# DIAGNijmegen/bodyct-dram-emph-subtype

Measured on NVIDIA B200. Metric: CT volumes/sec med3ddram inference, higher is better.
Workload: dtype f16 operands / f32 accumulate

## Files before the change

### bodyct-dram-emph-subtype_b200/_capi.py

```python
import ctypes as C
import os

HERE = os.path.dirname(os.path.abspath(__file__))
LIB_PATH = os.environ.get("DRAM_B200_LIB") or os.path.join(HERE, "libdram_b200.so")

DRAM_OK = 0
DRAM_DTYPE_BF16 = 0
DRAM_DTYPE_F16 = 1
CONV_ALGO = {"auto": 0, "tiles": 1, "planes": 2}
CONV_EPILOGUE = {"auto": 0, "direct": 1, "staged": 2}
LOSS_COEF_HEAD = 16
PEER_HANDLE_BYTES = 64


class ConvDesc(C.Structure):

    _fields_ = [
        ("n", C.c_int32), ("di", C.c_int32), ("hi", C.c_int32), ("wi", C.c_int32),
        ("c1", C.c_int32), ("c2", C.c_int32),
        ("cout", C.c_int32),
        ("kd", C.c_int32), ("kh", C.c_int32), ("kw", C.c_int32),
        ("sd", C.c_int32), ("sh", C.c_int32), ("sw", C.c_int32),
        ("dd", C.c_int32), ("dh", C.c_int32), ("dw", C.c_int32),
        ("pd", C.c_int32), ("ph", C.c_int32), ("pw", C.c_int32),
        ("relu", C.c_int32),
        ("res_c", C.c_int32), ("res_stride", C.c_int32),
        ("res_d", C.c_int32), ("res_h", C.c_int32), ("res_w", C.c_int32),
        ("n_heads", C.c_int32), ("head_ch", C.c_int32 * 2), ("head_sigmoid", C.c_int32),
        ("store_out", C.c_int32),
        ("tw", C.c_int32), ("th", C.c_int32), ("td", C.c_int32),
        ("dtype", C.c_int32),
        ("algo", C.c_int32),
        ("src1_up2x", C.c_int32),
        ("epilogue", C.c_int32),
    ]


_vp, _i32, _i64, _sz = C.c_void_p, C.c_int32, C.c_int64, C.c_size_t
_pi32 = C.POINTER(C.c_int32)

SIGNATURES = {
    "dram_version": (C.c_int, []),
    "dram_last_error": (C.c_int, [C.c_char_p, _sz]),
    "dram_sm_count": (C.c_int, []),
    "dram_set_saturation_counter": (C.c_int, [_vp]),
    "dram_conv3d_out_dims": (C.c_int, [C.POINTER(ConvDesc), _pi32, _pi32, _pi32]),
    "dram_conv3d_plan_create": (C.c_int, [C.POINTER(ConvDesc), _vp, _vp, _vp, _vp, _vp, _vp, _vp, _vp, _vp,
                                          _vp, _vp, C.POINTER(_vp)]),
    "dram_conv3d_plan_destroy": (C.c_int, [_vp]),
    "dram_conv3d_run": (C.c_int, [_vp, _i32, _vp]),
    "dram_conv3d_plan_info": (C.c_int, [_vp, C.POINTER(_i64), _pi32, _pi32, _pi32, _pi32]),
    "dram_conv3d_plan_executed_flops": (C.c_int, [_vp, C.POINTER(_i64)]),
    "dram_conv3d_worklist_size": (C.c_int, [_vp, _pi32]),
    "dram_conv3d_worklist": (C.c_int, [_vp, _vp, _i32, _vp, _vp, _vp, _vp]),
    "dram_conv3d_run_listed": (C.c_int, [_vp, _vp, _vp, _i32, _vp]),
    "dram_stem_expand": (C.c_int, [_vp, _vp, _i32, _i32, _i32, _i32, _i32, _vp]),
    "dram_stem_weight_bytes": (_sz, []),
    "dram_stem_conv7": (C.c_int, [_vp, _vp, _vp, _vp, _vp, _i32, _i32, _i32, _i32, _i32, _i32, _i32, _vp]),
    "dram_stem_conv7_hu": (C.c_int, [_vp, _vp, _i32, _i32, _vp, _vp, _vp, _vp, _i32, _i32, _i32, _i32, _i32, _i32,
                                     _i32, _vp]),
    "dram_maxpool3d": (C.c_int, [_vp, _vp, _i32, _i32, _i32, _i32, _i32, _i32, _vp]),
    "dram_upsample2x": (C.c_int, [_vp, _vp, _i32, _i32, _i32, _i32, _i32, _i32, _vp]),
    "dram_upsample2x_plan_create": (C.c_int, [_vp, _vp, _i32, _i32, _i32, _i32, _i32, _i32, C.POINTER(_vp)]),
    "dram_upsample2x_plan_destroy": (C.c_int, [_vp]),
    "dram_upsample2x_plan_run": (C.c_int, [_vp, _i32, _vp]),
    "dram_upsample2x_worklist_size": (C.c_int, [_vp, _pi32]),
    "dram_upsample2x_worklist": (C.c_int, [_vp, _vp, _i32, _vp, _vp, _vp, _vp]),
    "dram_upsample2x_plan_run_listed": (C.c_int, [_vp, _vp, _vp, _i32, _vp]),
    "dram_decoder_support": (C.c_int, [_vp, _i32, _i32, _i32, _i32, _i32, _i32, _i32, _vp, _vp, _vp]),
    "dram_upconv_axis": (C.c_int, [_vp, _vp, _i64, _i32, _i32, _i64, _i32, _i32, _i32, _vp]),
    "dram_pool_workspace_bytes": (_sz, [_i32, _i32]),
    "dram_masked_pool": (C.c_int, [_vp, _vp, _i32, _vp, _vp, _i32, _i32, _i32, _i32, _i32, _i32, _i32, _i32, _vp]),
    "dram_dram_workspace_bytes": (_sz, [_i32]),
    "dram_dram_upsample_mask": (C.c_int, [_vp, _vp, _vp, _vp, _vp, _vp, _vp, _vp, _i32, _i32, _i32, _i32,
                                          _i32, _i32, _i32, _i32, _vp]),
    "dram_lobe_workspace_bytes": (_sz, [_i32, _i64]),
    "dram_lobe_sums": (C.c_int, [_vp, _vp, _vp, _vp, _vp, _vp, _vp, _i32, _i64, _vp]),
    "dram_preprocess_workspace_bytes": (_sz, []),
    "dram_window_standardize": (C.c_int, [_vp, _vp, _vp, _vp, _i64, C.c_float, C.c_float, _vp]),
    "dram_preprocess_workspace_bytes_n": (_sz, [_i32]),
    "dram_window_standardize_batch": (C.c_int, [_vp, _vp, _vp, _vp, _i32, _i64, C.c_float, C.c_float, _vp]),
    "dram_window_stats": (C.c_int, [_vp, _vp, _vp, _i32, _i64, C.c_float, C.c_float, _vp]),
    "dram_window_lut": (C.c_int, [_vp, _vp, _vp, _vp, _i32, _i64, C.c_float, C.c_float, _vp]),
    "dram_resize_image": (C.c_int, [_vp, _vp, _vp, _i32, _i32, _i32, _i32, _i32, _i32, _vp]),
    "dram_resize_mask": (C.c_int, [_vp, _vp, _vp, _i32, _i32, _i32, _i32, _i32, _i32, _vp]),
    "dram_resize_labels": (C.c_int, [_vp, _vp, _vp, _i32, _i32, _i32, _i32, _i32, _i32, _vp]),
    "dram_mask_bbox": (C.c_int, [_vp, _i32, _i32, _i32, _vp, _vp]),
    "dram_lung_crop_workspace_bytes": (_sz, [_i32, _i32, _i32]),
    "dram_lung_crop": (C.c_int, [_vp, _vp, _i32, _i32, _i32, _i32, _i32, _i32, _i32, _i32, _i32, _vp, _vp, _vp, _vp, _vp]),
    "dram_label_counts": (C.c_int, [_vp, _i64, _vp, _vp]),
    "dram_label_hu_hist": (C.c_int, [_vp, _vp, _i64, _vp, _i32, _vp, _vp, _vp]),
    "dram_heatmap_u8": (C.c_int, [_vp, _i32, _i32, _i32, _vp, _i32, _i32, _i32, _i32, _i32, _i32, _i32, _i32, _i32, _vp]),
    "dram_conv3d_wgrad_workspace_bytes": (_i64, [C.POINTER(ConvDesc)]),
    "dram_conv3d_wgrad_plan_create": (C.c_int, [C.POINTER(ConvDesc), _vp, _vp, _vp, _i32, _i32, _vp, _i64, C.POINTER(_vp)]),
    "dram_conv3d_wgrad_plan_destroy": (C.c_int, [_vp]),
    "dram_conv3d_wgrad_plan_info": (C.c_int, [_vp, C.POINTER(_i64), _pi32, _pi32, _pi32]),
    "dram_conv3d_wgrad_run": (C.c_int, [_vp, _i32, _i32, _vp]),
    "dram_bn_workspace_bytes": (_i64, [_i32]),
    "dram_bn_stats": (C.c_int, [_vp, _i64, _i32, _i32, _vp, _vp, _vp]),
    "dram_bn_finalize": (C.c_int, [_vp, C.c_double, _vp, _vp, C.c_float, C.c_float, _vp, _vp, _vp, _vp, _vp, _vp, _i32, _vp]),
    "dram_bn_apply": (C.c_int, [_vp, _vp, _vp, _vp, _i32, _vp, _i64, _i32, _i32, _vp]),
    "dram_bn_backward_reduce": (C.c_int, [_vp, _vp, _vp, _vp, _vp, _i64, _i32, _i32, _vp, _vp, _vp]),
    "dram_bn_backward_apply": (C.c_int, [_vp, _vp, _vp, _vp, _vp, _vp, _vp, C.c_double, _vp, _vp, _i64, _i32, _i32, _vp]),
    "dram_upsample2x_backward": (C.c_int, [_vp, _vp, _i32, _i32, _i32, _i32, _i32, _i32, _vp]),
    "dram_maxpool3d_backward_workspace_bytes": (_i64, [_i32, _i32, _i32, _i32, _i32]),
    "dram_maxpool3d_backward": (C.c_int, [_vp, _vp, _vp, _vp, _i32, _i32, _i32, _i32, _i32, _i32, _vp]),
    "dram_heads_workspace_bytes": (_i64, []),
    "dram_heads_sigmoid_forward": (C.c_int, [_vp, _vp, _vp, _vp, _vp, _i64, _i32, _vp]),
    "dram_heads_sigmoid_backward": (C.c_int, [_vp, _vp, _vp, _vp, _vp, _vp, _vp, _vp, _vp, _vp, _i64, _i32, _vp]),
    "dram_peer_exchange_bytes": (_i64, []),
    "dram_peer_alloc": (C.c_int, [_i64, C.POINTER(_vp), _vp]),
    "dram_peer_open": (C.c_int, [_vp, C.POINTER(_vp)]),
    "dram_peer_close": (C.c_int, [_vp]),
    "dram_peer_free": (C.c_int, [_vp]),
    "dram_peer_allreduce_f64": (C.c_int, [_vp, _vp, _i32, _vp, _i32, _i32, C.c_uint64, _vp, _vp]),
    "dram_train_loss_workspace_bytes": (_i64, [_i32]),
    "dram_train_loss_forward": (C.c_int, [_vp, _vp, _vp, _vp, _vp, _vp, _vp, _vp, _vp, _vp, _i32, _i32, _i32, _i32, _i32,
                                          _i32, _i32, C.c_float, C.c_float, _vp, _vp, _vp]),
    "dram_train_loss_backward": (C.c_int, [_vp, _vp, _vp, _vp, _vp, _vp, _vp, _vp, _i32, _i32, _i32, _i32, _i32, _i32,
                                           _i32, _vp, _vp, _vp]),
    "dram_adam_step": (C.c_int, [_vp, _vp, _vp, _vp, _i64, C.c_double, C.c_double, C.c_double, C.c_double, _i32,
                                 C.c_float, _vp]),
    "dram_pack_conv_weight": (C.c_int, [_vp, _vp, _i32, _i32, _i32, _i32, _i32, _i32, _i32, _i32, _vp]),
    "dram_ncdhw_f32_to_ndhwc_16": (C.c_int, [_vp, _vp, _i32, _i32, _i32, _i32, _i32, _i32, _vp]),
    "dram_ndhwc_16_to_ncdhw_f32": (C.c_int, [_vp, _vp, _i32, _i32, _i32, _i32, _i32, _i32, _vp]),
}

_lib = None


class DramError(RuntimeError):
    """A libdram_b200 call returned a negative status."""


def load():
    global _lib
    if _lib is not None:
        return _lib
    if not os.path.exists(LIB_PATH):
        raise ImportError(
            f"{LIB_PATH} is missing: build it with `python {os.path.join(HERE, 'build.py')}` "
            "(there is no CPU or library fallback for this path)")
    lib = C.CDLL(LIB_PATH)
    for name, (res, args) in SIGNATURES.items():
        fn = getattr(lib, name)
        fn.restype = res
        fn.argtypes = args
    _lib = lib
    return lib


def last_error():
    buf = C.create_string_buffer(512)
    load().dram_last_error(buf, len(buf))
    return buf.value.decode("utf-8", "replace")


def check(status, what):
    if status != DRAM_OK:
        raise DramError(f"{what} failed ({status}): {last_error()}")
```

### bodyct-dram-emph-subtype_b200/csrc/conv3d_pair.cu

```cuda
#include "conv_plan.h"

namespace dram {

static constexpr int P_BLOCK_N = 256;
static constexpr int P_BLOCK_K = 64;
static constexpr int P_A_BYTES = 128 * P_BLOCK_K * 2;
static constexpr int P_B_BYTES = P_BLOCK_N * P_BLOCK_K * 2;
static constexpr int P_STAGE_BYTES = 2 * P_A_BYTES + P_B_BYTES;
static constexpr int P_STAGES = 3;
static constexpr int P_THREADS = 320;
static constexpr int P_PRODUCER_WARP = 4, P_MMA_WARP = 5;
static constexpr int P_TMEM_COLS = 512;
static constexpr int P_SMEM_BYTES = 1024 + P_STAGES * P_STAGE_BYTES + 256;

struct PairCoord {
  TileCoord t[2];
  bool m_ok[2];
};
__device__ __forceinline__ PairCoord decode_pair(const ConvKParams &p, int tile) {
  PairCoord pc;
  const int n_tile = tile % p.num_n_tiles;
  const int pair = tile / p.num_n_tiles;
#pragma unroll
  for (int b = 0; b < 2; ++b) {
    const int m_tile = 2 * pair + b;
    pc.m_ok[b] = m_tile < p.m_tiles_total;
    pc.t[b] = decode_tile(p, m_tile * p.num_n_tiles + n_tile, P_BLOCK_N);
  }
  return pc;
}
__device__ __forceinline__ bool brick_tap_is_padding(const ConvKParams &p, const TileCoord &t, int zd, int zh, int zw) {
  return tap_is_padding(t.d0 * p.sd + zd * p.dd - p.pd, p.td, p.sd, p.Di) ||
         tap_is_padding(t.h0 * p.sh + zh * p.dh - p.ph, p.th, p.sh, p.Hi) ||
         tap_is_padding(t.w0 * p.sw + zw * p.dw - p.pw, p.tw, p.sw, p.Wi);
}

__global__ void __launch_bounds__(P_THREADS, 1)
conv3d_pair_kernel(const __grid_constant__ CUtensorMap map_a1, const __grid_constant__ CUtensorMap map_a2,
                   const __grid_constant__ CUtensorMap map_w, const __grid_constant__ ConvKParams p) {
  extern __shared__ uint8_t smem_raw[];
  const uint32_t smem_base = (smem_u32(smem_raw) + 1023u) & ~1023u;
  const uint32_t bar_base = smem_base + P_STAGES * P_STAGE_BYTES;
  auto full_bar = [&](int s) { return bar_base + 8u * s; };
  auto empty_bar = [&](int s) { return bar_base + 8u * (P_STAGES + s); };
  const uint32_t tmem_full_bar = bar_base + 8u * (2 * P_STAGES);
  const uint32_t tmem_empty_bar = bar_base + 8u * (2 * P_STAGES + 1);
  const uint32_t tmem_slot = bar_base + 8u * (2 * P_STAGES + 2);
  auto smem_a = [&](int s, int b) { return smem_base + (uint32_t)(s * P_STAGE_BYTES + b * P_A_BYTES); };
  auto smem_b = [&](int s) { return smem_base + (uint32_t)(s * P_STAGE_BYTES + 2 * P_A_BYTES); };

  const int warp = uniform_warp_idx();
  const int lane = threadIdx.x & 31;

  if (threadIdx.x == 0) {
    for (int s = 0; s < P_STAGES; ++s) {
      mbar_init(full_bar(s), 1);
      mbar_init(empty_bar(s), 1);
    }
    mbar_init(tmem_full_bar, 1);
    mbar_init(tmem_empty_bar, 256);
    asm volatile("fence.mbarrier_init.release.cluster;" ::: "memory");
  }
  if (warp == P_MMA_WARP) tmem_alloc(tmem_slot, P_TMEM_COLS);
  if (warp == P_PRODUCER_WARP && lane == 0) {
    prefetch_tensormap(&map_a1);
    prefetch_tensormap(&map_a2);
    prefetch_tensormap(&map_w);
  }
  tcgen05_fence_before();
  __syncthreads();
  tcgen05_fence_after();
  uint32_t tmem_base;
  asm volatile("ld.shared.b32 %0, [%1];" : "=r"(tmem_base) : "r"(tmem_slot));
  tmem_base = __shfl_sync(0xffffffffu, tmem_base, 0);

  if (warp == P_PRODUCER_WARP) {
    if (lane == 0) {
      int stage = 0;
      uint32_t phase = 0;
      for (int tile = blockIdx.x; tile < p.total_tiles; tile += gridDim.x) {
        const PairCoord pc = decode_pair(p, tile);
        for (int zd = 0; zd < p.kd; ++zd)
          for (int zh = 0; zh < p.kh; ++zh)
            for (int zw = 0; zw < p.kw; ++zw) {
              if (brick_tap_is_padding(p, pc.t[0], zd, zh, zw) && brick_tap_is_padding(p, pc.t[1], zd, zh, zw)) continue;
              const int tap = (zd * p.kh + zh) * p.kw + zw;
              for (int ch = 0; ch < p.chunks_total; ++ch) {
                mbar_wait(empty_bar(stage), phase ^ 1u);
                mbar_expect_tx(full_bar(stage), P_STAGE_BYTES);
#pragma unroll
                for (int b = 0; b < 2; ++b) {
                  const TileCoord &t = pc.t[b];
                  const int iw0 = t.w0 * p.sw + zw * p.dw - p.pw, ih0 = t.h0 * p.sh + zh * p.dh - p.ph;
                  const int id0 = t.d0 * p.sd + zd * p.dd - p.pd;
                  if (ch < p.chunks1)
                    tma_load_5d(smem_a(stage, b), &map_a1, full_bar(stage), ch * P_BLOCK_K, iw0, ih0, id0, t.sample);
                  else
                    tma_load_5d(smem_a(stage, b), &map_a2, full_bar(stage), (ch - p.chunks1) * P_BLOCK_K, iw0, ih0,
                                id0, t.sample);
                }
                tma_load_2d(smem_b(stage), &map_w, full_bar(stage), (tap * p.chunks_total + ch) * P_BLOCK_K,
                            pc.t[0].n0);
                if (++stage == P_STAGES) {
                  stage = 0;
                  phase ^= 1u;
                }
              }
            }
      }
    }
    __syncwarp();
  } else if (warp == P_MMA_WARP) {
    const uint32_t idesc = make_idesc_16bit(128, P_BLOCK_N, p.epi.is_f16);
    int stage = 0;
    uint32_t phase = 0, acc_phase = 0;
    for (int tile = blockIdx.x; tile < p.total_tiles; tile += gridDim.x) {
      const PairCoord pc = decode_pair(p, tile);
      mbar_wait(tmem_empty_bar, acc_phase ^ 1u);
      tcgen05_fence_after();
      uint32_t accumulate = 0;
      for (int zd = 0; zd < p.kd; ++zd)
        for (int zh = 0; zh < p.kh; ++zh)
          for (int zw = 0; zw < p.kw; ++zw) {
            if (brick_tap_is_padding(p, pc.t[0], zd, zh, zw) && brick_tap_is_padding(p, pc.t[1], zd, zh, zw)) continue;
            for (int ch = 0; ch < p.chunks_total; ++ch) {
              mbar_wait(full_bar(stage), phase);
              tcgen05_fence_after();
              const uint64_t da0 = make_sw128_desc(smem_a(stage, 0)), da1 = make_sw128_desc(smem_a(stage, 1));
              const uint64_t db = make_sw128_desc(smem_b(stage));
              if (elect_one_sync()) {
#pragma unroll
                for (int k = 0; k < 4; ++k) {
                  umma_bf16(tmem_base, da0 + (uint64_t)(2 * k), db + (uint64_t)(2 * k), idesc, (k > 0) ? 1u : accumulate);
                  umma_bf16(tmem_base + P_BLOCK_N, da1 + (uint64_t)(2 * k), db + (uint64_t)(2 * k), idesc,
                            (k > 0) ? 1u : accumulate);
                }
                umma_commit(empty_bar(stage));
              }
              __syncwarp();
              accumulate = 1;
              if (++stage == P_STAGES) {
                stage = 0;
                phase ^= 1u;
              }
            }
          }
      if (elect_one_sync()) umma_commit(tmem_full_bar);
      __syncwarp();
      acc_phase ^= 1u;
    }
  } else {
    const int quarter = warp & 3, brick = warp < 4 ? 0 : 1;
    const int row = quarter * 32 + lane;
    const int lw = row & (p.tw - 1);
    const int lh = (row >> p.tw_log2) & (p.th - 1);
    const int ld = row >> (p.tw_log2 + p.th_log2);
    uint32_t acc_phase = 0;
    for (int tile = blockIdx.x; tile < p.total_tiles; tile += gridDim.x) {
      const PairCoord pc = decode_pair(p, tile);
      const TileCoord &t = pc.t[brick];
      const int od = t.d0 + ld, oh = t.h0 + lh, ow = t.w0 + lw;
      const bool valid = pc.m_ok[brick] && (od < p.Do) && (oh < p.Ho) && (ow < p.Wo);
      const uint16_t *res_row = residual_row(p.epi, valid, t.sample, od, oh, ow);
      mbar_wait(tmem_full_bar, acc_phase);
      tcgen05_fence_after();
      const uint32_t taddr = tmem_base + (uint32_t)(brick * P_BLOCK_N) + ((uint32_t)(quarter * 32) << 16);
      ResGroup res = load_residual_group(p.epi, res_row, t.n0);
#pragma unroll 1
      for (int c0 = 0; c0 < P_BLOCK_N; c0 += 32) {
        uint32_t v[32];
        tmem_ld_32x32b_x32(taddr + (uint32_t)c0, v);
        const ResGroup next = load_residual_group(p.epi, c0 + 32 < P_BLOCK_N ? res_row : nullptr, t.n0 + c0 + 32);
        tmem_wait_ld();
        if (valid) epilogue_group<false>(p.epi, v, t.n0 + c0, t.sample, od, oh, ow, res);
        res = next;
      }
      tcgen05_fence_before();
      mbar_arrive(tmem_empty_bar);
      acc_phase ^= 1u;
    }
  }

  tcgen05_fence_before();
  __syncthreads();
  if (warp == P_MMA_WARP) {
    tcgen05_fence_after();
    tmem_dealloc(tmem_base, P_TMEM_COLS);
  }
}

int pair_plan_wanted(const dram_conv_desc *d, int block_n, int64_t k_chunks, int64_t m_tiles, int n_tiles) {
  if (!(block_n == P_BLOCK_N && d->cout % P_BLOCK_N == 0 && k_chunks >= 64 && d->n_heads == 0 && d->store_out))
    return 0;
  const char *knob = getenv("DRAM_B200_PAIR_TILES");
  if (knob) return atoi(knob) != 0;
  const int64_t pair_tiles = (m_tiles + 1) / 2 * n_tiles;
  return k_chunks >= 200 && pair_tiles >= 6LL * sm_count();
}

int pair_plan_fill(dram_conv_plan *pl) {
  ConvKParams &p = pl->p;
  p.m_tiles_total = pl->m_tiles;
  const int64_t total = (int64_t)((pl->m_tiles + 1) / 2) * p.num_n_tiles;
  p.total_tiles = (int)total;
  pl->pair = 1;
  pl->stages = P_STAGES;
  pl->smem_bytes = P_SMEM_BYTES;
  return check_cuda(cudaFuncSetAttribute(conv3d_pair_kernel, cudaFuncAttributeMaxDynamicSharedMemorySize, P_SMEM_BYTES),
                    "cudaFuncSetAttribute(conv3d_pair_kernel)");
}

int pair_plan_run(const dram_conv_plan *pl, int ctas, cudaStream_t st) {
  if (pl->p.total_tiles < ctas) ctas = pl->p.total_tiles;
  ConvKParams kp = pl->p;
  kp.epi = with_sat_counter(kp.epi);
  conv3d_pair_kernel<<<ctas, P_THREADS, pl->smem_bytes, st>>>(pl->map_a1, pl->map_a2, pl->map_w, kp);
  DRAM_CHECK_LAUNCH("conv3d_pair_kernel launch");
  return DRAM_OK;
}

}
```

### bodyct-dram-emph-subtype_b200/csrc/conv3d_umma.cu

```cuda
#include "umma_common.cuh"
#include "conv_plan.h"

namespace dram {

static constexpr int BLOCK_M = 128;
static constexpr int BLOCK_K = 64;
static constexpr int UMMA_K = 16;
static constexpr int A_STAGE_BYTES = BLOCK_M * BLOCK_K * 2;
static constexpr int NUM_THREADS = 192;
static constexpr int NUM_THREADS_STAGED = 320;
static constexpr int PRODUCER_WARP = 4;
static constexpr int MMA_WARP = 5;

static constexpr int EPI_TILE_BYTES = BLOCK_M * 128;
static constexpr int RES_BUFS = 4;

template <int BLOCK_N, bool STAGED = false>
struct ConvCfg {
  static constexpr int B_STAGE_BYTES = BLOCK_N * BLOCK_K * 2;
  static constexpr int STAGE_BYTES = A_STAGE_BYTES + B_STAGE_BYTES;
  static constexpr int STAGES = STAGED ? (BLOCK_N == 256 ? 3 : 4) : ((BLOCK_N <= 64) ? 8 : (BLOCK_N == 128 ? 6 : 4));
  static constexpr int TMEM_COLS = (2 * BLOCK_N < 32) ? 32 : 2 * BLOCK_N;
  static constexpr int RES_TILES = BLOCK_N == 256 ? 0 : RES_BUFS;
  static constexpr int EPI_BYTES = STAGED ? (2 + RES_TILES) * EPI_TILE_BYTES : 0;
  static constexpr int SMEM_BYTES = 1024 + STAGES * STAGE_BYTES + EPI_BYTES + 256;
};

template <int BLOCK_N, bool STAGED>
__global__ void __launch_bounds__(STAGED ? NUM_THREADS_STAGED : NUM_THREADS, 1)
conv3d_umma_kernel(const __grid_constant__ CUtensorMap map_a1,
                   const __grid_constant__ CUtensorMap map_a2,
                   const __grid_constant__ CUtensorMap map_w, const __grid_constant__ CUtensorMap map_out,
                   const __grid_constant__ CUtensorMap map_res, const __grid_constant__ ConvKParams p) {
  using Cfg = ConvCfg<BLOCK_N, STAGED>;
  constexpr int STAGES = Cfg::STAGES;
  extern __shared__ uint8_t smem_raw[];
  const uint32_t smem_base = (smem_u32(smem_raw) + 1023u) & ~1023u;
  const uint32_t epi_base = smem_base + STAGES * Cfg::STAGE_BYTES;
  const uint32_t bar_base = epi_base + Cfg::EPI_BYTES;
  auto out_tile = [&](int b) { return epi_base + (uint32_t)b * EPI_TILE_BYTES; };
  auto res_tile = [&](int b) { return epi_base + (uint32_t)(2 + b) * EPI_TILE_BYTES; };
  auto res_full = [&](int q, int b) { return bar_base + 8u * (2 * STAGES + 5 + q * RES_BUFS + b); };
  auto full_bar = [&](int s) { return bar_base + 8u * s; };
  auto empty_bar = [&](int s) { return bar_base + 8u * (STAGES + s); };
  auto tmem_full_bar = [&](int a) { return bar_base + 8u * (2 * STAGES + a); };
  auto tmem_empty_bar = [&](int a) { return bar_base + 8u * (2 * STAGES + 2 + a); };
  const uint32_t tmem_slot = bar_base + 8u * (2 * STAGES + 4);
  auto smem_a = [&](int s) { return smem_base + s * Cfg::STAGE_BYTES; };
  auto smem_b = [&](int s) { return smem_base + s * Cfg::STAGE_BYTES + A_STAGE_BYTES; };

  const int warp = uniform_warp_idx();
  const int lane = threadIdx.x & 31;

  if (threadIdx.x == 0) {
    for (int s = 0; s < STAGES; ++s) {
      mbar_init(full_bar(s), 1);
      mbar_init(empty_bar(s), 1);
    }
    for (int a = 0; a < 2; ++a) {
      mbar_init(tmem_full_bar(a), 1);
      mbar_init(tmem_empty_bar(a), STAGED ? 256 : 128);
    }
    if (STAGED)
      for (int b = 0; b < 4 * RES_BUFS; ++b) mbar_init(res_full(0, b), 1);
    asm volatile("fence.mbarrier_init.release.cluster;" ::: "memory");
  }
  if (warp == MMA_WARP) tmem_alloc(tmem_slot, Cfg::TMEM_COLS);
  if (warp == PRODUCER_WARP && lane == 0) {
    prefetch_tensormap(&map_a1);
    prefetch_tensormap(&map_a2);
    prefetch_tensormap(&map_w);
  }
  if (STAGED && threadIdx.x == 0) {
    prefetch_tensormap(&map_out);
    prefetch_tensormap(&map_res);
  }
  tcgen05_fence_before();
  __syncthreads();
  tcgen05_fence_after();
  uint32_t tmem_base;
  asm volatile("ld.shared.b32 %0, [%1];" : "=r"(tmem_base) : "r"(tmem_slot));
  tmem_base = __shfl_sync(0xffffffffu, tmem_base, 0);

  if (warp == PRODUCER_WARP) {
    if (lane == 0) {
      int stage = 0;
      uint32_t phase = 0;
      for (int tile = blockIdx.x; tile < p.total_tiles; tile += gridDim.x) {
        const TileCoord t = decode_tile(p, tile, BLOCK_N);
        for (int zd = 0; zd < p.kd; ++zd) {
          const int id0 = t.d0 * p.sd + zd * p.dd - p.pd;
          if (tap_is_padding(id0, p.td, p.sd, p.Di)) continue;
          for (int zh = 0; zh < p.kh; ++zh) {
            const int ih0 = t.h0 * p.sh + zh * p.dh - p.ph;
            if (tap_is_padding(ih0, p.th, p.sh, p.Hi)) continue;
            for (int zw = 0; zw < p.kw; ++zw) {
              const int iw0 = t.w0 * p.sw + zw * p.dw - p.pw;
              if (tap_is_padding(iw0, p.tw, p.sw, p.Wi)) continue;
              const int tap = (zd * p.kh + zh) * p.kw + zw;
              for (int ch = 0; ch < p.chunks_total; ++ch) {
                mbar_wait(empty_bar(stage), phase ^ 1u);
                mbar_expect_tx(full_bar(stage), Cfg::STAGE_BYTES);
                if (ch < p.chunks1)
                  tma_load_5d(smem_a(stage), &map_a1, full_bar(stage), ch * BLOCK_K, iw0, ih0, id0,
                              t.sample);
                else
                  tma_load_5d(smem_a(stage), &map_a2, full_bar(stage), (ch - p.chunks1) * BLOCK_K,
                              iw0, ih0, id0, t.sample);
                tma_load_2d(smem_b(stage), &map_w, full_bar(stage),
                            (tap * p.chunks_total + ch) * BLOCK_K, t.n0);
                if (++stage == STAGES) {
                  stage = 0;
                  phase ^= 1u;
                }
              }
            }
          }
        }
      }
    }
    __syncwarp();
  } else if (warp == MMA_WARP) {
    {
      const uint32_t idesc = make_idesc_16bit(BLOCK_M, BLOCK_N, p.epi.is_f16);
      int stage = 0;
      uint32_t phase = 0;
      int acc = 0;
      uint32_t acc_phase = 0;
      for (int tile = blockIdx.x; tile < p.total_tiles; tile += gridDim.x) {
        const TileCoord t = decode_tile(p, tile, BLOCK_N);
        mbar_wait(tmem_empty_bar(acc), acc_phase ^ 1u);
        tcgen05_fence_after();
        const uint32_t tmem_d = tmem_base + (uint32_t)(acc * BLOCK_N);
        uint32_t accumulate = 0;
        for (int zd = 0; zd < p.kd; ++zd) {
          if (tap_is_padding(t.d0 * p.sd + zd * p.dd - p.pd, p.td, p.sd, p.Di)) continue;
          for (int zh = 0; zh < p.kh; ++zh) {
            if (tap_is_padding(t.h0 * p.sh + zh * p.dh - p.ph, p.th, p.sh, p.Hi)) continue;
            for (int zw = 0; zw < p.kw; ++zw) {
              if (tap_is_padding(t.w0 * p.sw + zw * p.dw - p.pw, p.tw, p.sw, p.Wi)) continue;
              for (int ch = 0; ch < p.chunks_total; ++ch) {
                mbar_wait(full_bar(stage), phase);
                tcgen05_fence_after();
                const uint64_t da = make_sw128_desc(smem_a(stage));
                const uint64_t db = make_sw128_desc(smem_b(stage));
                if (elect_one_sync()) {
#pragma unroll
                  for (int k = 0; k < BLOCK_K / UMMA_K; ++k) {
                    umma_bf16(tmem_d, da + (uint64_t)(2 * k), db + (uint64_t)(2 * k), idesc,
                              (k > 0) ? 1u : accumulate);
                  }
                  umma_commit(empty_bar(stage));
                }
                __syncwarp();
                accumulate = 1;
                if (++stage == STAGES) {
                  stage = 0;
                  phase ^= 1u;
                }
              }
            }
          }
        }
        if (elect_one_sync()) umma_commit(tmem_full_bar(acc));
        __syncwarp();
        if (++acc == 2) {
          acc = 0;
          acc_phase ^= 1u;
        }
      }
    }
    __syncwarp();
  } else if (STAGED) {
    constexpr int GROUPS = BLOCK_N >= 64 ? BLOCK_N / 64 : 1;
    constexpr uint32_t SLICE_BYTES = EPI_TILE_BYTES / 4;
    const int quarter = warp & 3, half = warp < 4 ? 0 : 1;
    const int row = quarter * 32 + lane;
    const bool storer = half == 0 && lane == 0;
    const int row0 = quarter * 32;
    const int qw = row0 & (p.tw - 1), qh = (row0 >> p.tw_log2) & (p.th - 1), qd = row0 >> (p.tw_log2 + p.th_log2);
    const bool has_res = p.staged_res != 0;
    const int my_tiles = p.total_tiles > (int)blockIdx.x ? (p.total_tiles - 1 - (int)blockIdx.x) / (int)gridDim.x + 1 : 0;
    const int total_groups = my_tiles * GROUPS;
    auto pair_sync = [&]() { asm volatile("bar.sync %0, 64;" ::"r"(1 + quarter) : "memory"); };
    auto issue_res = [&](int gi) {
      if (!has_res || gi >= total_groups) return;
      const int tile = blockIdx.x + (gi / GROUPS) * gridDim.x;
      const TileCoord t = decode_tile(p, tile, BLOCK_N);
      const int rb = gi % RES_BUFS;
      mbar_expect_tx(res_full(quarter, rb), SLICE_BYTES);
      const int rs = p.epi.res_stride;
      tma_load_5d(res_tile(rb) + (uint32_t)quarter * SLICE_BYTES, &map_res, res_full(quarter, rb),
                  t.n0 + (gi % GROUPS) * 64, (t.w0 + qw) * rs, (t.h0 + qh) * rs, (t.d0 + qd) * rs, t.sample);
    };
    if (storer)
      for (int g0 = 0; g0 < RES_BUFS; ++g0) issue_res(g0);
    int acc = 0, gi = 0;
    uint32_t acc_phase = 0;
    for (int tile = blockIdx.x; tile < p.total_tiles; tile += gridDim.x) {
      const TileCoord t = decode_tile(p, tile, BLOCK_N);
      mbar_wait(tmem_full_bar(acc), acc_phase);
      tcgen05_fence_after();
      const uint32_t taddr = tmem_base + (uint32_t)(acc * BLOCK_N) + ((uint32_t)(quarter * 32) << 16);
#pragma unroll 1
      for (int g = 0; g < GROUPS; ++g, ++gi) {
        const int b = gi & 1, rb = gi % RES_BUFS;
        uint32_t v[32];
        tmem_ld_32x32b_x32(taddr + (uint32_t)(g * 64 + half * 32), v);
        if (has_res) mbar_wait(res_full(quarter, rb), (uint32_t)((gi / RES_BUFS) & 1));
        if (storer) tma_store_wait_read<1>();
        pair_sync();
        tmem_wait_ld();
        epilogue_group_staged(p.epi, v, t.n0 + g * 64 + half * 32, row, half, res_tile(rb), has_res, out_tile(b));
        asm volatile("fence.proxy.async.shared::cta;" ::: "memory");
        pair_sync();
        if (storer) {
          if (t.w0 + qw < p.Wo && t.h0 + qh < p.Ho && t.d0 + qd < p.Do)
            tma_store_5d(&map_out, out_tile(b) + (uint32_t)quarter * SLICE_BYTES, t.n0 + g * 64, t.w0 + qw, t.h0 + qh,
                         t.d0 + qd, t.sample);
          tma_store_commit();
          issue_res(gi + RES_BUFS);
        }
      }
      tcgen05_fence_before();
      mbar_arrive(tmem_empty_bar(acc));
      if (++acc == 2) {
        acc = 0;
        acc_phase ^= 1u;
      }
    }
    if (storer) asm volatile("cp.async.bulk.wait_group 0;" ::: "memory");
  } else {
    const int row = warp * 32 + lane;
    const int lw = row & (p.tw - 1);
    const int lh = (row >> p.tw_log2) & (p.th - 1);
    const int ld = row >> (p.tw_log2 + p.th_log2);
    int acc = 0;
    uint32_t acc_phase = 0;
    for (int tile = blockIdx.x; tile < p.total_tiles; tile += gridDim.x) {
      const TileCoord t = decode_tile(p, tile, BLOCK_N);
      const int od = t.d0 + ld, oh = t.h0 + lh, ow = t.w0 + lw;
      const bool valid = (od < p.Do) && (oh < p.Ho) && (ow < p.Wo);
      const uint16_t *res_row = residual_row(p.epi, valid, t.sample, od, oh, ow);
      ResGroup res = load_residual_group(p.epi, res_row, t.n0);
      mbar_wait(tmem_full_bar(acc), acc_phase);
      tcgen05_fence_after();
      const uint32_t taddr = tmem_base + (uint32_t)(acc * BLOCK_N) + ((uint32_t)(warp * 32) << 16);
#pragma unroll 1
      for (int c0 = 0; c0 < BLOCK_N; c0 += 32) {
        uint32_t v[32];
        tmem_ld_32x32b_x32(taddr + (uint32_t)c0, v);
        const ResGroup next = load_residual_group(p.epi, c0 + 32 < BLOCK_N ? res_row : nullptr, t.n0 + c0 + 32);
        tmem_wait_ld();
        if (valid) epilogue_group<BLOCK_N == 32>(p.epi, v, t.n0 + c0, t.sample, od, oh, ow, res);
        res = next;
      }
      tcgen05_fence_before();
      mbar_arrive(tmem_empty_bar(acc));
      if (++acc == 2) {
        acc = 0;
        acc_phase ^= 1u;
      }
    }
  }

  tcgen05_fence_before();
  __syncthreads();
  if (warp == MMA_WARP) {
    tcgen05_fence_after();
    tmem_dealloc(tmem_base, Cfg::TMEM_COLS);
  }
}

typedef CUresult (*EncodeTiledFn)(CUtensorMap *, CUtensorMapDataType, cuuint32_t, void *,
                                  const cuuint64_t *, const cuuint64_t *, const cuuint32_t *,
                                  const cuuint32_t *, CUtensorMapInterleave, CUtensorMapSwizzle,
                                  CUtensorMapL2promotion, CUtensorMapFloatOOBfill);

static EncodeTiledFn get_encode_fn() {
  static EncodeTiledFn fn = nullptr;
  if (fn) return fn;
  void *sym = nullptr;
  cudaDriverEntryPointQueryResult q;
  cudaError_t e = cudaGetDriverEntryPoint("cuTensorMapEncodeTiled", &sym, cudaEnableDefault, &q);
  if (e != cudaSuccess || q != cudaDriverEntryPointSuccess || sym == nullptr) {
    cudaGetLastError();
    return nullptr;
  }
  fn = reinterpret_cast<EncodeTiledFn>(sym);
  return fn;
}

int encode_act_map(CUtensorMap *map, const void *base, int n, int d, int h, int w, int c, int box_c, int bw,
                   int bh, int bd, int sw, int sh, int sd, int is_f16) {
  EncodeTiledFn enc = get_encode_fn();
  if (!enc) {
    set_error("cuTensorMapEncodeTiled is not available (no CUDA driver?)");
    return DRAM_E_DRIVER;
  }
  cuuint64_t gdim[5] = {(cuuint64_t)c, (cuuint64_t)w, (cuuint64_t)h, (cuuint64_t)d, (cuuint64_t)n};
  cuuint64_t gstr[4] = {(cuuint64_t)c * 2, (cuuint64_t)w * c * 2, (cuuint64_t)h * w * c * 2,
                        (cuuint64_t)d * h * w * c * 2};
  cuuint32_t box[5] = {(cuuint32_t)box_c, (cuuint32_t)((bw - 1) * sw + 1),
                       (cuuint32_t)((bh - 1) * sh + 1), (cuuint32_t)((bd - 1) * sd + 1), 1};
  cuuint32_t estr[5] = {1, (cuuint32_t)sw, (cuuint32_t)sh, (cuuint32_t)sd, 1};
  CUresult r = enc(map, is_f16 ? CU_TENSOR_MAP_DATA_TYPE_FLOAT16 : CU_TENSOR_MAP_DATA_TYPE_BFLOAT16, 5,
                   const_cast<void *>(base), gdim, gstr, box, estr, CU_TENSOR_MAP_INTERLEAVE_NONE,
                   CU_TENSOR_MAP_SWIZZLE_128B, CU_TENSOR_MAP_L2_PROMOTION_L2_256B,
                   CU_TENSOR_MAP_FLOAT_OOB_FILL_NONE);
  if (r != CUDA_SUCCESS) {
    set_error("cuTensorMapEncodeTiled(activation %dx%dx%dx%dx%d box %dx%dx%d stride %d,%d,%d) -> %d",
              n, d, h, w, c, bw, bh, bd, sw, sh, sd, (int)r);
    return DRAM_E_DRIVER;
  }
  return DRAM_OK;
}

int encode_act_map_plain(CUtensorMap *map, const void *base, int n, int d, int h, int w, int c, int box_c, int bw,
                         int bh, int is_f16) {
  EncodeTiledFn enc = get_encode_fn();
  if (!enc) {
    set_error("cuTensorMapEncodeTiled is not available (no CUDA driver?)");
    return DRAM_E_DRIVER;
  }
  cuuint64_t gdim[5] = {(cuuint64_t)c, (cuuint64_t)w, (cuuint64_t)h, (cuuint64_t)d, (cuuint64_t)n};
  cuuint64_t gstr[4] = {(cuuint64_t)c * 2, (cuuint64_t)w * c * 2, (cuuint64_t)h * w * c * 2,
                        (cuuint64_t)d * h * w * c * 2};
  cuuint32_t box[5] = {(cuuint32_t)box_c, (cuuint32_t)bw, (cuuint32_t)bh, 1, 1};
  cuuint32_t estr[5] = {1, 1, 1, 1, 1};
  CUresult r = enc(map, is_f16 ? CU_TENSOR_MAP_DATA_TYPE_FLOAT16 : CU_TENSOR_MAP_DATA_TYPE_BFLOAT16, 5,
                   const_cast<void *>(base), gdim, gstr, box, estr, CU_TENSOR_MAP_INTERLEAVE_NONE,
                   CU_TENSOR_MAP_SWIZZLE_NONE, CU_TENSOR_MAP_L2_PROMOTION_L2_256B, CU_TENSOR_MAP_FLOAT_OOB_FILL_NONE);
  if (r != CUDA_SUCCESS) {
    set_error("cuTensorMapEncodeTiled(plain activation %dx%dx%dx%dx%d box %dx%d) -> %d", n, d, h, w, c, bw, bh, (int)r);
    return DRAM_E_DRIVER;
  }
  return DRAM_OK;
}

int encode_weight_map(CUtensorMap *map, const void *base, int cout, int64_t ktot, int block_n, int is_f16) {
  EncodeTiledFn enc = get_encode_fn();
  if (!enc) {
    set_error("cuTensorMapEncodeTiled is not available (no CUDA driver?)");
    return DRAM_E_DRIVER;
  }
  cuuint64_t gdim[2] = {(cuuint64_t)ktot, (cuuint64_t)cout};
  cuuint64_t gstr[1] = {(cuuint64_t)ktot * 2};
  cuuint32_t box[2] = {(cuuint32_t)BLOCK_K, (cuuint32_t)block_n};
  cuuint32_t estr[2] = {1, 1};
  CUresult r = enc(map, is_f16 ? CU_TENSOR_MAP_DATA_TYPE_FLOAT16 : CU_TENSOR_MAP_DATA_TYPE_BFLOAT16, 2,
                   const_cast<void *>(base), gdim, gstr, box, estr, CU_TENSOR_MAP_INTERLEAVE_NONE,
                   CU_TENSOR_MAP_SWIZZLE_128B, CU_TENSOR_MAP_L2_PROMOTION_L2_256B,
                   CU_TENSOR_MAP_FLOAT_OOB_FILL_NONE);
  if (r != CUDA_SUCCESS) {
    set_error("cuTensorMapEncodeTiled(weight %d x %lld, box_n %d) -> %d", cout, (long long)ktot,
              block_n, (int)r);
    return DRAM_E_DRIVER;
  }
  return DRAM_OK;
}

static int ilog2(int v) {
  int l = 0;
  while ((1 << l) < v) ++l;
  return l;
}
static bool is_pow2(int v) { return v > 0 && (v & (v - 1)) == 0; }

static int conv_out(int in, int k, int s, int d, int p) { return (in + 2 * p - d * (k - 1) - 1) / s + 1; }

int pair_plan_wanted(const dram_conv_desc *d, int block_n, int64_t k_chunks, int64_t m_tiles, int n_tiles);
int pair_plan_fill(dram_conv_plan *pl);
int pair_plan_run(const dram_conv_plan *pl, int ctas, cudaStream_t st);

int slab_plan_supported(const dram_conv_desc *d);
int slab_plan_fill(dram_conv_plan *pl, const dram_conv_desc *d, const void *src1, const void *src2,
                   const void *weight, const EpiParams &epi);
int slab_plan_run(const dram_conv_plan *pl, int ctas, cudaStream_t st, const int *items, const int *count);
int slab_plan_listable(const dram_conv_plan *pl);
int slab_plan_worklist(const dram_conv_plan *pl, const uint32_t *bits, int radius, uint8_t *flags, int *list, int *count,
                       cudaStream_t st);

}

using namespace dram;

extern "C" int dram_conv3d_out_dims(const dram_conv_desc *d, int32_t *dout, int32_t *hout,
                                    int32_t *wout) {
  DRAM_REQUIRE(d && dout && hout && wout, "dram_conv3d_out_dims: null argument");
  DRAM_REQUIRE(d->sd > 0 && d->sh > 0 && d->sw > 0, "dram_conv3d_out_dims: stride must be positive");
  *dout = conv_out(d->di, d->kd, d->sd, d->dd, d->pd);
  *hout = conv_out(d->hi, d->kh, d->sh, d->dh, d->ph);
  *wout = conv_out(d->wi, d->kw, d->sw, d->dw, d->pw);
  return DRAM_OK;
}

template <int BN, bool STAGED>
static int set_smem_attr() {
  return check_cuda(cudaFuncSetAttribute(conv3d_umma_kernel<BN, STAGED>,
                                         cudaFuncAttributeMaxDynamicSharedMemorySize,
                                         ConvCfg<BN, STAGED>::SMEM_BYTES),
                    "cudaFuncSetAttribute(conv3d_umma_kernel)");
}
template <int BN, bool STAGED>
static int fill_tile_cfg(dram_conv_plan *pl) {
  pl->stages = ConvCfg<BN, STAGED>::STAGES;
  pl->smem_bytes = ConvCfg<BN, STAGED>::SMEM_BYTES;
  return set_smem_attr<BN, STAGED>();
}
template <int BN, bool STAGED>
static void launch_tiles(const dram_conv_plan *pl, dim3 grid, cudaStream_t st) {
  ConvKParams kp = pl->p;
  kp.epi = with_sat_counter(kp.epi);
  conv3d_umma_kernel<BN, STAGED><<<grid, STAGED ? NUM_THREADS_STAGED : NUM_THREADS, pl->smem_bytes, st>>>(
      pl->map_a1, pl->map_a2, pl->map_w, pl->map_out, pl->map_res, kp);
}

extern "C" int dram_conv3d_plan_create(const dram_conv_desc *d, const void *src1, const void *src2,
                                       const void *weight, const float *bias, const float *scale,
                                       const void *residual, void *out, const float *head_w,
                                       const float *head_b, float *head_out0, float *head_out1,
                                       dram_conv_plan **plan) {
  DRAM_REQUIRE(d && plan, "dram_conv3d_plan_create: null descriptor or plan pointer");
  *plan = nullptr;
  DRAM_REQUIRE(src1 && weight && bias, "dram_conv3d_plan_create: src1, weight and bias are required");
  DRAM_REQUIRE(d->n > 0 && d->di > 0 && d->hi > 0 && d->wi > 0, "conv3d: empty input");
  DRAM_REQUIRE(d->c1 > 0 && d->c1 % 64 == 0, "conv3d: c1=%d must be a positive multiple of 64", d->c1);
  DRAM_REQUIRE(d->c2 >= 0 && d->c2 % 64 == 0, "conv3d: c2=%d must be a multiple of 64", d->c2);
  DRAM_REQUIRE((d->c2 == 0) == (src2 == nullptr), "conv3d: src2 must be given exactly when c2 > 0");
  DRAM_REQUIRE(d->cout > 0 && d->cout % 32 == 0, "conv3d: cout=%d must be a multiple of 32", d->cout);
  DRAM_REQUIRE(d->kd >= 1 && d->kh >= 1 && d->kw >= 1 && d->kd <= 7 && d->kh <= 7 && d->kw <= 7,
               "conv3d: filter extent must be in 1..7");
  DRAM_REQUIRE(d->sd >= 1 && d->sh >= 1 && d->sw >= 1 && d->sd <= 8 && d->sh <= 8 && d->sw <= 8,
               "conv3d: stride must be in 1..8");
  DRAM_REQUIRE(d->dd >= 1 && d->dh >= 1 && d->dw >= 1, "conv3d: dilation must be >= 1");
  DRAM_REQUIRE(d->pd >= 0 && d->ph >= 0 && d->pw >= 0, "conv3d: padding must be >= 0");
  DRAM_REQUIRE(d->dtype == DRAM_DTYPE_BF16 || d->dtype == DRAM_DTYPE_F16, "conv3d: dtype must be bf16 (0) or fp16 (1)");
  DRAM_REQUIRE(d->algo >= DRAM_CONV_ALGO_AUTO && d->algo <= DRAM_CONV_ALGO_PLANES, "conv3d: bad algo %d", d->algo);
  DRAM_REQUIRE(d->epilogue >= DRAM_CONV_EPILOGUE_AUTO && d->epilogue <= DRAM_CONV_EPILOGUE_STAGED, "conv3d: bad epilogue %d",
               d->epilogue);
  DRAM_REQUIRE(d->store_out == 0 || out != nullptr, "conv3d: out is required when store_out != 0");
  DRAM_REQUIRE(d->store_out != 0 || d->n_heads > 0, "conv3d: nothing to write");

  int Do, Ho, Wo;
  dram_conv3d_out_dims(d, &Do, &Ho, &Wo);
  DRAM_REQUIRE(Do > 0 && Ho > 0 && Wo > 0, "conv3d: empty output");

  int block_n;
  if (d->cout % 256 == 0) block_n = 256;
  else if (d->cout % 128 == 0) block_n = 128;
  else if (d->cout % 64 == 0) block_n = 64;
  else block_n = 32;
  if (d->cout == 32) block_n = 32;
  DRAM_REQUIRE(d->cout % block_n == 0, "conv3d: cout=%d is not tileable", d->cout);

  if (d->n_heads > 0) {
    DRAM_REQUIRE(d->cout == 32, "conv3d: fused heads need cout == 32 (got %d)", d->cout);
    DRAM_REQUIRE(d->n_heads <= 2 && head_w && head_b && head_out0, "conv3d: bad head arguments");
    DRAM_REQUIRE(d->head_ch[0] >= 1 && (d->n_heads == 1 || (d->head_ch[1] >= 1 && head_out1)),
                 "conv3d: bad head channel counts");
    DRAM_REQUIRE(d->head_ch[0] + (d->n_heads == 2 ? d->head_ch[1] : 0) <= 16,
                 "conv3d: at most 16 head channels");
  }
  if (d->res_c > 0) {
    DRAM_REQUIRE(residual != nullptr, "conv3d: res_c > 0 but residual is NULL");
    DRAM_REQUIRE(d->res_c % 32 == 0 && d->res_c <= d->cout, "conv3d: res_c=%d must be a multiple of 32 and <= cout", d->res_c);
    DRAM_REQUIRE(d->res_stride >= 1, "conv3d: res_stride must be >= 1");
    DRAM_REQUIRE((Do - 1) * d->res_stride < d->res_d && (Ho - 1) * d->res_stride < d->res_h &&
                     (Wo - 1) * d->res_stride < d->res_w,
                 "conv3d: residual tensor %dx%dx%d too small for output %dx%dx%d at stride %d",
                 d->res_d, d->res_h, d->res_w, Do, Ho, Wo, d->res_stride);
  }

  EpiParams epi;
  memset(&epi, 0, sizeof(epi));
  epi.Do = Do; epi.Ho = Ho; epi.Wo = Wo;
  epi.cout = d->cout;
  epi.relu = d->relu;
  epi.is_f16 = d->dtype == DRAM_DTYPE_F16;
  epi.bias = bias;
  epi.scale = scale;
  epi.out = reinterpret_cast<uint16_t *>(out);
  epi.res = d->res_c > 0 ? reinterpret_cast<const uint16_t *>(residual) : nullptr;
  epi.res_c = d->res_c; epi.res_stride = d->res_stride > 0 ? d->res_stride : 1;
  epi.res_d = d->res_d; epi.res_h = d->res_h; epi.res_w = d->res_w;
  epi.n_heads = d->n_heads;
  epi.head_ch0 = d->n_heads > 0 ? d->head_ch[0] : 0;
  epi.head_ch1 = d->n_heads > 1 ? d->head_ch[1] : 0;
  epi.head_sigmoid = d->head_sigmoid;
  epi.store_out = d->store_out;
  epi.head_w = head_w; epi.head_b = head_b; epi.head_out0 = head_out0; epi.head_out1 = head_out1;

  const int taps = d->kd * d->kh * d->kw;
  const int64_t ktot = (int64_t)taps * (d->c1 + d->c2);

  dram_conv_plan *pl = new dram_conv_plan();
  memset(pl, 0, sizeof(*pl));
  pl->flops = 2LL * d->n * Do * Ho * Wo * (int64_t)d->cout * ktot;
  pl->block_n = block_n;

  const bool want_planes = d->algo == DRAM_CONV_ALGO_PLANES ||
                           (d->algo == DRAM_CONV_ALGO_AUTO && d->tw == 0 && slab_plan_supported(d));
  if (d->src1_up2x && !(want_planes && slab_plan_supported(d))) {
    delete pl;
    set_error("conv3d: src1_up2x is implemented by the plane-ring kernel only (3x3x3, stride 1, dilation 1, cout 64)");
    return DRAM_E_ARG;
  }
  if (want_planes) {
    if (!slab_plan_supported(d)) {
      delete pl;
      set_error("conv3d: DRAM_CONV_ALGO_PLANES needs a 3x3x3 stride-1 dilation-1 pad-1 filter and cout of 32 or 64");
      return DRAM_E_ARG;
    }
    int rc = slab_plan_fill(pl, d, src1, src2, weight, epi);
    if (rc != DRAM_OK) {
      delete pl;
      return rc;
    }
    *plan = pl;
    return DRAM_OK;
  }

  int tw = d->tw, th = d->th, td = d->td;
  if (tw == 0 || th == 0 || td == 0) {
    static const int cand[][3] = {{8, 4, 4}, {4, 8, 4}, {4, 4, 8}, {8, 8, 2},  {8, 2, 8}, {2, 8, 8},
                                  {16, 4, 2}, {4, 16, 2}, {16, 2, 4}, {2, 16, 4}, {16, 8, 1}, {8, 16, 1},
                                  {32, 4, 1}, {4, 32, 1}, {32, 2, 2}, {16, 1, 8}, {128, 1, 1}};
    int64_t best = -1;
    for (auto &c : cand) {
      int64_t tiles = (int64_t)ceil_div(Wo, c[0]) * ceil_div(Ho, c[1]) * ceil_div(Do, c[2]);
      if (best < 0 || tiles < best) {
        best = tiles;
        tw = c[0];
        th = c[1];
        td = c[2];
      }
    }
  }
  if (!(is_pow2(tw) && is_pow2(th) && is_pow2(td) && tw * th * td == BLOCK_M)) {
    delete pl;
    set_error("conv3d: tile %dx%dx%d must be powers of two with product 128", tw, th, td);
    return DRAM_E_ARG;
  }
  if (!((tw - 1) * d->sw + 1 <= 256 && (th - 1) * d->sh + 1 <= 256 && (td - 1) * d->sd + 1 <= 256)) {
    delete pl;
    set_error("conv3d: TMA box too large for tile/stride");
    return DRAM_E_ARG;
  }

  pl->kind = 0;
  ConvKParams &p = pl->p;
  p.n = d->n; p.Do = Do; p.Ho = Ho; p.Wo = Wo; p.Di = d->di; p.Hi = d->hi; p.Wi = d->wi;
  p.tw = tw; p.th = th; p.td = td; p.tw_log2 = ilog2(tw); p.th_log2 = ilog2(th);
  p.tiles_w = ceil_div(Wo, tw); p.tiles_h = ceil_div(Ho, th); p.tiles_d = ceil_div(Do, td);
  p.tiles_per_sample = p.tiles_w * p.tiles_h * p.tiles_d;
  p.num_n_tiles = d->cout / block_n;
  int64_t total = (int64_t)p.tiles_per_sample * d->n * p.num_n_tiles;
  if (total > 0x7fffffffLL) {
    delete pl;
    set_error("conv3d: too many tiles");
    return DRAM_E_ARG;
  }
  p.total_tiles = (int)total;
  p.kd = d->kd; p.kh = d->kh; p.kw = d->kw; p.sd = d->sd; p.sh = d->sh; p.sw = d->sw;
  p.dd = d->dd; p.dh = d->dh; p.dw = d->dw; p.pd = d->pd; p.ph = d->ph; p.pw = d->pw;
  p.chunks1 = d->c1 / BLOCK_K;
  p.chunks_total = (d->c1 + d->c2) / BLOCK_K;
  p.epi = epi;
  pl->m_tiles = p.tiles_per_sample * d->n;
  pl->n_tiles = p.num_n_tiles;

  int rc = encode_act_map(&pl->map_a1, src1, d->n, d->di, d->hi, d->wi, d->c1, BLOCK_K, tw, th, td, d->sw,
                          d->sh, d->sd, epi.is_f16);
  if (rc == DRAM_OK) {
    if (d->c2 > 0)
      rc = encode_act_map(&pl->map_a2, src2, d->n, d->di, d->hi, d->wi, d->c2, BLOCK_K, tw, th, td, d->sw,
                          d->sh, d->sd, epi.is_f16);
    else
      pl->map_a2 = pl->map_a1;
  }
  if (rc == DRAM_OK) rc = encode_weight_map(&pl->map_w, weight, d->cout, ktot, block_n, epi.is_f16);
  const bool res_tma = d->res_c % 64 == 0;
  const char *stg = getenv("DRAM_B200_STAGED_EPILOGUE");
  const bool staged_ok = taps == 1 && block_n >= 64 && d->store_out && d->n_heads == 0 && (d->res_c == 0 || res_tma);
  if (d->epilogue == DRAM_CONV_EPILOGUE_STAGED && !staged_ok) {
    delete pl;
    set_error("conv3d: the staged epilogue needs a 1x1x1 filter, cout %% 64 == 0, a stored output, no heads and res_c %% 64 == 0");
    return DRAM_E_ARG;
  }
  pl->staged = staged_ok && d->epilogue != DRAM_CONV_EPILOGUE_DIRECT &&
               (d->epilogue == DRAM_CONV_EPILOGUE_STAGED || !(stg && atoi(stg) == 0));
  const bool staged256 = pl->staged && block_n == 256 && d->res_c == 0 && d->epilogue == DRAM_CONV_EPILOGUE_STAGED;
  if (pl->staged && block_n > 128 && !staged256) {
    block_n = 128;
    pl->block_n = block_n;
    p.num_n_tiles = d->cout / block_n;
    const int64_t total2 = (int64_t)p.tiles_per_sample * d->n * p.num_n_tiles;
    if (total2 > 0x7fffffffLL) {
      delete pl;
      set_error("conv3d: too many tiles");
      return DRAM_E_ARG;
    }
    p.total_tiles = (int)total2;
    pl->n_tiles = p.num_n_tiles;
    rc = rc == DRAM_OK ? encode_weight_map(&pl->map_w, weight, d->cout, ktot, block_n, epi.is_f16) : rc;
  }
  p.staged_res = pl->staged && d->res_c > 0;
  pl->map_out = pl->map_a1;
  pl->map_res = pl->map_a1;
  if (rc == DRAM_OK && pl->staged) {
    const int qbw = tw < 32 ? tw : 32, qbh = (32 / qbw) < th ? 32 / qbw : th, qbd = 32 / (qbw * qbh);
    rc = encode_act_map(&pl->map_out, out, d->n, Do, Ho, Wo, d->cout, 64, qbw, qbh, qbd, 1, 1, 1, epi.is_f16);
    if (rc == DRAM_OK && p.staged_res)
      rc = encode_act_map(&pl->map_res, residual, d->n, d->res_d, d->res_h, d->res_w, d->res_c, 64, qbw, qbh, qbd,
                          epi.res_stride, epi.res_stride, epi.res_stride, epi.is_f16);
  }
  if (rc == DRAM_OK) {
    if (pl->staged) {
      switch (block_n) {
        case 64: rc = fill_tile_cfg<64, true>(pl); break;
        case 256: rc = fill_tile_cfg<256, true>(pl); break;
        default: rc = fill_tile_cfg<128, true>(pl); break;
      }
    } else if (d->tw == 0 && pair_plan_wanted(d, block_n, (int64_t)taps * p.chunks_total, pl->m_tiles, pl->n_tiles)) {
      rc = pair_plan_fill(pl);
    } else {
      switch (block_n) {
        case 32: rc = fill_tile_cfg<32, false>(pl); break;
        case 64: rc = fill_tile_cfg<64, false>(pl); break;
        case 128: rc = fill_tile_cfg<128, false>(pl); break;
        default: rc = fill_tile_cfg<256, false>(pl); break;
      }
    }
  }
  if (rc != DRAM_OK) {
    delete pl;
    return rc;
  }
  *plan = pl;
  return DRAM_OK;
}

extern "C" int dram_conv3d_plan_destroy(dram_conv_plan *plan) {
  delete plan;
  return DRAM_OK;
}

extern "C" int dram_conv3d_plan_info(const dram_conv_plan *plan, int64_t *flops, int32_t *m_tiles,
                                     int32_t *n_tiles, int32_t *block_n, int32_t *stages) {
  DRAM_REQUIRE(plan, "dram_conv3d_plan_info: null plan");
  if (flops) *flops = plan->flops;
  if (m_tiles) *m_tiles = plan->m_tiles;
  if (n_tiles) *n_tiles = plan->n_tiles;
  if (block_n) *block_n = plan->block_n;
  if (stages) *stages = plan->kind == 1 ? -plan->stages : plan->stages;
  return DRAM_OK;
}

static bool host_tap_is_padding(int i0, int extent, int stride, int in_size) {
  return (i0 + (extent - 1) * stride < 0) || (i0 >= in_size);
}
static bool host_brick_tap_skipped(const ConvKParams &p, int m_tile, int zd, int zh, int zw) {
  const int r = m_tile % p.tiles_per_sample;
  const int iw = r % p.tiles_w, r2 = r / p.tiles_w, ih = r2 % p.tiles_h, id = r2 / p.tiles_h;
  return host_tap_is_padding(id * p.td * p.sd + zd * p.dd - p.pd, p.td, p.sd, p.Di) ||
         host_tap_is_padding(ih * p.th * p.sh + zh * p.dh - p.ph, p.th, p.sh, p.Hi) ||
         host_tap_is_padding(iw * p.tw * p.sw + zw * p.dw - p.pw, p.tw, p.sw, p.Wi);
}

extern "C" int dram_conv3d_plan_executed_flops(const dram_conv_plan *plan, int64_t *flops) {
  DRAM_REQUIRE(plan && flops, "dram_conv3d_plan_executed_flops: null argument");
  if (plan->kind == 1) {
    const SlabParams &sp = plan->sp;
    if (sp.stream) {
      const int64_t cols = (int64_t)sp.n * sp.cols_w * sp.cols_h;
      *flops = 2LL * cols * (3LL * sp.D - 2) * 128 * 32 * 9 * 64;
      return DRAM_OK;
    }
    const int group = plan->block_n == 128 ? 2 : 4;
    *flops = 2LL * sp.items_total * group * 128 * (int64_t)plan->block_n * 27 * sp.chunks_total * 64;
    return DRAM_OK;
  }
  const ConvKParams &p = plan->p;
  const int m_tiles = plan->m_tiles;
  int64_t stages = 0;
  if (plan->pair) {
    for (int pr = 0; 2 * pr < m_tiles; ++pr)
      for (int zd = 0; zd < p.kd; ++zd)
        for (int zh = 0; zh < p.kh; ++zh)
          for (int zw = 0; zw < p.kw; ++zw) {
            const bool s0 = host_brick_tap_skipped(p, 2 * pr, zd, zh, zw);
            const bool s1 = 2 * pr + 1 < m_tiles ? host_brick_tap_skipped(p, 2 * pr + 1, zd, zh, zw) : true;
            if (!(s0 && s1)) stages += 2;
          }
  } else {
    for (int m = 0; m < m_tiles; ++m)
      for (int zd = 0; zd < p.kd; ++zd)
        for (int zh = 0; zh < p.kh; ++zh)
          for (int zw = 0; zw < p.kw; ++zw)
            if (!host_brick_tap_skipped(p, m, zd, zh, zw)) ++stages;
  }
  *flops = 2LL * stages * p.num_n_tiles * 128 * (int64_t)plan->block_n * p.chunks_total * 64;
  return DRAM_OK;
}

extern "C" int dram_conv3d_run(const dram_conv_plan *plan, int32_t max_ctas, void *stream) {
  DRAM_REQUIRE(plan, "dram_conv3d_run: null plan");
  int ctas = sm_count();
  if (max_ctas > 0 && max_ctas < ctas) ctas = max_ctas;
  cudaStream_t st = reinterpret_cast<cudaStream_t>(stream);
  if (plan->kind == 1) return slab_plan_run(plan, ctas, st, nullptr, nullptr);
  if (plan->pair) return pair_plan_run(plan, ctas, st);
  if (plan->p.total_tiles < ctas) ctas = plan->p.total_tiles;
  dim3 grid(ctas);
  if (plan->staged) {
    switch (plan->block_n) {
      case 64: launch_tiles<64, true>(plan, grid, st); break;
      case 256: launch_tiles<256, true>(plan, grid, st); break;
      default: launch_tiles<128, true>(plan, grid, st); break;
    }
  } else {
    switch (plan->block_n) {
      case 32: launch_tiles<32, false>(plan, grid, st); break;
      case 64: launch_tiles<64, false>(plan, grid, st); break;
      case 128: launch_tiles<128, false>(plan, grid, st); break;
      default: launch_tiles<256, false>(plan, grid, st); break;
    }
  }
  DRAM_CHECK_LAUNCH("conv3d_umma_kernel launch");
  return DRAM_OK;
}

static bool conv_listable(const dram_conv_plan *plan) { return plan->kind == 1 && slab_plan_listable(plan); }

extern "C" int dram_conv3d_worklist_size(const dram_conv_plan *plan, int32_t *entries) {
  DRAM_REQUIRE(plan && entries, "dram_conv3d_worklist_size: null argument");
  *entries = conv_listable(plan) ? (plan->sp.stream ? plan->sp.steps_total : plan->sp.items_total) : 0;
  return DRAM_OK;
}

extern "C" int dram_conv3d_worklist(const dram_conv_plan *plan, const uint32_t *support, int32_t radius, uint8_t *flags,
                                    int32_t *items, int32_t *count, void *stream) {
  DRAM_REQUIRE(plan, "dram_conv3d_worklist: null plan");
  DRAM_REQUIRE(conv_listable(plan), "dram_conv3d_worklist: this plan's kernel takes no work list");
  return slab_plan_worklist(plan, support, radius, flags, items, count, reinterpret_cast<cudaStream_t>(stream));
}

extern "C" int dram_conv3d_run_listed(const dram_conv_plan *plan, const int32_t *items, const int32_t *count,
                                      int32_t max_ctas, void *stream) {
  DRAM_REQUIRE(plan && items && count, "dram_conv3d_run_listed: null argument");
  DRAM_REQUIRE(conv_listable(plan), "dram_conv3d_run_listed: this plan's kernel takes no work list");
  int ctas = sm_count();
  if (max_ctas > 0 && max_ctas < ctas) ctas = max_ctas;
  return slab_plan_run(plan, ctas, reinterpret_cast<cudaStream_t>(stream), items, count);
}
```

### bodyct-dram-emph-subtype_b200/csrc/conv_plan.h

```cpp
#pragma once
#include "umma_common.cuh"

namespace dram {

struct ConvKParams {
  int n, Do, Ho, Wo, Di, Hi, Wi;
  int tw, th, td;
  int tw_log2, th_log2;
  int tiles_w, tiles_h, tiles_d, tiles_per_sample, num_n_tiles, total_tiles;
  int kd, kh, kw, sd, sh, sw, dd, dh, dw, pd, ph, pw;
  int chunks1, chunks_total;
  int staged_res;
  int m_tiles_total;
  EpiParams epi;
};


#ifdef __CUDACC__
struct TileCoord {
  int n0, sample, d0, h0, w0;
};
__device__ __forceinline__ TileCoord decode_tile(const ConvKParams &p, int tile, int block_n) {
  TileCoord t;
  int n_tile = tile % p.num_n_tiles;
  int m_tile = tile / p.num_n_tiles;
  t.n0 = n_tile * block_n;
  t.sample = m_tile / p.tiles_per_sample;
  int r = m_tile - t.sample * p.tiles_per_sample;
  int iw = r % p.tiles_w;
  int r2 = r / p.tiles_w;
  int ih = r2 % p.tiles_h;
  int id = r2 / p.tiles_h;
  t.w0 = iw * p.tw;
  t.h0 = ih * p.th;
  t.d0 = id * p.td;
  return t;
}
__device__ __forceinline__ bool tap_is_padding(int i0, int extent, int stride, int in_size) {
  return (i0 + (extent - 1) * stride < 0) || (i0 >= in_size);
}
#endif

struct SlabParams {
  int n, D, H, W;
  int cols_w, cols_h, groups_d, items_total;
  int chunks1, chunks_total;
  int desc_base_offset_mode;
  int up2x;
  int Dl, Hl, Wl;
  float up_sd, up_sh, up_sw;
  int stream;
  int steps_total;
  const int *items, *count;
  EpiParams epi;
};

}

struct dram_conv_plan {
  int kind;
  CUtensorMap map_a1, map_a2, map_w;
  CUtensorMap map_out, map_res;
  int staged;
  int pair;
  dram::ConvKParams p;
  dram::SlabParams sp;
  int block_n;
  int stages;
  size_t smem_bytes;
  int64_t flops;
  int m_tiles, n_tiles;
};
```

### bodyct-dram-emph-subtype_b200/ops.py

```python
import ctypes as C
import os

import torch

from . import _capi
from ._capi import ConvDesc, check

ACT_DTYPES = {torch.bfloat16: _capi.DRAM_DTYPE_BF16, torch.float16: _capi.DRAM_DTYPE_F16}


def default_act_dtype():
    name = os.environ.get("DRAM_B200_DTYPE", "fp16").lower()
    if name in ("fp16", "f16", "float16", "half"):
        return torch.float16
    if name in ("bf16", "bfloat16"):
        return torch.bfloat16
    raise ValueError(f"DRAM_B200_DTYPE={name!r}: expected fp16 or bf16")


class ActivationOverflow(RuntimeError):
    """A convolution output left the finite fp16 range and was clamped (see dram_set_saturation_counter)."""


def sat_check_mode():
    mode = os.environ.get("DRAM_B200_SAT_CHECK", "first").lower()
    if mode not in ("first", "always", "off"):
        raise ValueError(f"DRAM_B200_SAT_CHECK={mode!r}: expected first, always or off")
    return mode


def graphs_enabled():
    return os.environ.get("DRAM_B200_GRAPH", "1").lower() not in ("0", "off", "false", "no")


def _need16(t, name, ndim=None):
    if isinstance(t, torch.Tensor) and t.dtype not in ACT_DTYPES:
        raise TypeError(f"{name}: expected bfloat16 or float16, got {t.dtype}")
    return _need(t, t.dtype, name, ndim)


def _stream():
    return C.c_void_p(torch.cuda.current_stream().cuda_stream)


def _p(t):
    return None if t is None else C.c_void_p(t.data_ptr())


def _need(t, dtype, name, ndim=None):
    if not isinstance(t, torch.Tensor) or not t.is_cuda:
        raise RuntimeError(f"{name}: expected a CUDA tensor (libdram_b200 has no CPU fallback)")
    if t.dtype != dtype:
        raise TypeError(f"{name}: expected dtype {dtype}, got {t.dtype}")
    if not t.is_contiguous():
        raise ValueError(f"{name}: tensor must be contiguous")
    if ndim is not None and t.dim() != ndim:
        raise ValueError(f"{name}: expected {ndim} dims, got shape {tuple(t.shape)}")
    return t


def sm_count():
    return _capi.load().dram_sm_count()


def _triple(v):
    return (v, v, v) if isinstance(v, int) else tuple(v)


class Conv3dPlan:

    def __init__(self, x1, weight, bias, *, x2=None, scale=None, kernel=3, stride=1, dilation=1,
                 padding=None, relu=True, residual=None, res_stride=1, heads=None, store_out=True,
                 out=None, tile=None, algo="auto", upsample_x1=False, epilogue="auto"):
        lib = _capi.load()
        _need16(x1, "conv3d x1", 5)
        adt = x1.dtype
        n, di, hi, wi, c1 = x1.shape
        if upsample_x1:
            di, hi, wi = 2 * di, 2 * hi, 2 * wi
        c2 = 0
        if x2 is not None:
            _need(x2, adt, "conv3d x2", 5)
            if tuple(x2.shape[:4]) != (n, di, hi, wi):
                raise ValueError(f"conv3d: x2 {tuple(x2.shape)} does not match x1 {tuple(x1.shape)}")
            c2 = x2.shape[4]
        k, s, dl = _triple(kernel), _triple(stride), _triple(dilation)
        pad = tuple(dl[i] * (k[i] - 1) // 2 for i in range(3)) if padding is None else _triple(padding)
        _need(weight, adt, "conv3d weight", 2)
        _need(bias, torch.float32, "conv3d bias", 1)
        if scale is not None:
            _need(scale, torch.float32, "conv3d scale", 1)
            if scale.shape[0] != weight.shape[0]:
                raise ValueError("conv3d: scale length != cout")
        cout = weight.shape[0]
        taps = k[0] * k[1] * k[2]
        if weight.shape[1] != taps * (c1 + c2):
            raise ValueError(f"conv3d: packed weight K={weight.shape[1]} != taps*(c1+c2)={taps * (c1 + c2)}")
        if bias.shape[0] != cout:
            raise ValueError("conv3d: bias length != cout")

        d = ConvDesc()
        d.n, d.di, d.hi, d.wi, d.c1, d.c2, d.cout = n, di, hi, wi, c1, c2, cout
        d.kd, d.kh, d.kw = k
        d.sd, d.sh, d.sw = s
        d.dd, d.dh, d.dw = dl
        d.pd, d.ph, d.pw = pad
        d.relu = 1 if relu else 0
        d.dtype = ACT_DTYPES[adt]
        d.algo = _capi.CONV_ALGO[algo]
        d.src1_up2x = 1 if upsample_x1 else 0
        d.epilogue = _capi.CONV_EPILOGUE[epilogue]
        if residual is not None:
            _need(residual, adt, "conv3d residual", 5)
            d.res_c = residual.shape[4]
            d.res_stride = res_stride
            d.res_d, d.res_h, d.res_w = residual.shape[1:4]
            if residual.shape[0] != n:
                raise ValueError("conv3d: residual batch mismatch")
        else:
            d.res_stride = 1
        head_w = head_b = None
        if heads is not None:
            head_w, head_b, head_ch, sigmoid = heads
            _need(head_w, torch.float32, "conv3d head_w", 2)
            _need(head_b, torch.float32, "conv3d head_b", 1)
            d.n_heads = len(head_ch)
            for i, ch in enumerate(head_ch):
                d.head_ch[i] = ch
            d.head_sigmoid = 1 if sigmoid else 0
            if head_w.shape != (sum(head_ch), 32) or head_b.shape[0] != sum(head_ch):
                raise ValueError("conv3d: head weight/bias shape mismatch")
        d.store_out = 1 if store_out else 0
        if tile is not None:
            d.tw, d.th, d.td = tile

        do, ho, wo = C.c_int32(), C.c_int32(), C.c_int32()
        check(lib.dram_conv3d_out_dims(C.byref(d), C.byref(do), C.byref(ho), C.byref(wo)), "dram_conv3d_out_dims")
        self.out_shape = (n, do.value, ho.value, wo.value, cout)
        if store_out:
            if out is None:
                out = torch.empty(self.out_shape, dtype=adt, device=x1.device)
            else:
                _need(out, adt, "conv3d out", 5)
                if tuple(out.shape) != self.out_shape:
                    raise ValueError(f"conv3d: out shape {tuple(out.shape)} != {self.out_shape}")
        else:
            out = None
        self.out = out
        self.head_outs = []
        if heads is not None:
            for ch in heads[2]:
                self.head_outs.append(torch.empty((n, ch, do.value, ho.value, wo.value), dtype=torch.float32,
                                                  device=x1.device))
        ho0 = self.head_outs[0] if len(self.head_outs) > 0 else None
        ho1 = self.head_outs[1] if len(self.head_outs) > 1 else None

        handle = C.c_void_p()
        check(lib.dram_conv3d_plan_create(C.byref(d), _p(x1), _p(x2), _p(weight), _p(bias), _p(scale),
                                          _p(residual), _p(out), _p(head_w), _p(head_b), _p(ho0), _p(ho1),
                                          C.byref(handle)), "dram_conv3d_plan_create")
        self._handle = handle
        self._lib = lib
        self._keep = (x1, x2, weight, bias, scale, residual, out, head_w, head_b, ho0, ho1)
        flops, mt, nt, bn, st = C.c_int64(), C.c_int32(), C.c_int32(), C.c_int32(), C.c_int32()
        check(lib.dram_conv3d_plan_info(handle, C.byref(flops), C.byref(mt), C.byref(nt), C.byref(bn),
                                        C.byref(st)), "dram_conv3d_plan_info")
        self.flops, self.m_tiles, self.n_tiles, self.block_n, self.stages = (
            flops.value, mt.value, nt.value, bn.value, abs(st.value))
        self.algo = "planes" if st.value < 0 else "tiles"
        ex = C.c_int64()
        check(lib.dram_conv3d_plan_executed_flops(handle, C.byref(ex)), "dram_conv3d_plan_executed_flops")
        self.executed_flops = ex.value
        self.desc = d

    def run(self, max_ctas=0):
        check(self._lib.dram_conv3d_run(self._handle, max_ctas, _stream()), "dram_conv3d_run")
        return self.out

    def worklist_size(self):
        n = C.c_int32()
        check(self._lib.dram_conv3d_worklist_size(self._handle, C.byref(n)), "dram_conv3d_worklist_size")
        return n.value

    def build_worklist(self, support, radius, flags, items, count):
        check(self._lib.dram_conv3d_worklist(self._handle, _p(support), radius, _p(flags), _p(items), _p(count),
                                             _stream()), "dram_conv3d_worklist")

    def run_listed(self, items, count, max_ctas=0):
        check(self._lib.dram_conv3d_run_listed(self._handle, _p(items), _p(count), max_ctas, _stream()),
              "dram_conv3d_run_listed")
        return self.out

    def __del__(self):
        h = getattr(self, "_handle", None)
        if h:
            try:
                self._lib.dram_conv3d_plan_destroy(h)
            except Exception:
                pass
            self._handle = None


def pow2_normalizer(w2d):
    amax = w2d.abs().amax(dim=1).clamp_min(2.0 ** -100)
    return torch.exp2(torch.floor(torch.log2(amax)) + 1.0)


def pack_conv_weight(weight, scale=None, dtype=torch.bfloat16, normalize=False):
    w = weight.detach().to(torch.float32)
    if scale is not None:
        w = w * scale.to(torch.float32).view(-1, 1, 1, 1, 1)
    cout = w.shape[0]
    w = w.permute(0, 2, 3, 4, 1).reshape(cout, -1)
    if normalize:
        mult = pow2_normalizer(w)
        return (w / mult.view(-1, 1)).to(dtype).contiguous(), mult.contiguous()
    return w.to(dtype).contiguous()


def fold_bn(bn, conv_bias=None, eps=None):
    eps = bn.eps if eps is None else eps
    scale = bn.weight.detach().float() / torch.sqrt(bn.running_var.detach().float() + eps)
    shift = bn.bias.detach().float() - bn.running_mean.detach().float() * scale
    if conv_bias is not None:
        shift = shift + conv_bias.detach().float() * scale
    return scale, shift


def stem_expand(x, out=None, dtype=torch.bfloat16):
    _need(x, torch.float32, "stem_expand x", 4)
    n, d, h, w = x.shape
    shape = (n, d, (h - 1) // 2 + 1, (w - 1) // 2 + 1, 64)
    if out is None:
        out = torch.empty(shape, dtype=dtype, device=x.device)
    _need16(out, "stem_expand out", 5)
    check(_capi.load().dram_stem_expand(_p(x), _p(out), n, d, h, w, ACT_DTYPES[out.dtype], _stream()),
          "dram_stem_expand")
    return out


def pack_stem_weight(weight, scale=None, dtype=torch.bfloat16, normalize=False):
    w = weight.detach().to(torch.float32)
    if scale is not None:
        w = w * scale.to(torch.float32).view(-1, 1, 1, 1, 1)
    cout = w.shape[0]
    packed = torch.zeros((cout, 7, 8, 8), dtype=torch.float32, device=w.device)
    packed[:, :, :7, :7] = w[:, 0]
    packed = packed.reshape(cout, 7 * 64)
    if normalize:
        mult = pow2_normalizer(packed)
        return (packed / mult.view(-1, 1)).to(dtype).contiguous(), mult.contiguous()
    return packed.to(dtype).contiguous()


def pack_stem_weight_fused(weight, scale=None, dtype=torch.bfloat16, normalize=False):
    w = weight.detach().to(torch.float32)
    if scale is not None:
        w = w * scale.to(torch.float32).view(-1, 1, 1, 1, 1)
    cout = w.shape[0]
    if tuple(w.shape) != (64, 1, 7, 7, 7):
        raise ValueError(f"pack_stem_weight_fused: expected conv1.weight [64,1,7,7,7], got {tuple(w.shape)}")
    mult = pow2_normalizer(w.reshape(cout, -1)) if normalize else None
    if normalize:
        w = w / mult.view(-1, 1, 1, 1, 1)
    full = torch.zeros((7, 8, cout, 8), dtype=torch.float32, device=w.device)
    full[:, :7, :, 1:] = w[:, 0].permute(1, 2, 0, 3)
    even = full[[6, 4, 2, 0]].permute(1, 0, 2, 3)
    odd = full[[5, 3, 1]].permute(1, 0, 2, 3)
    packed = torch.cat([even.reshape(-1), odd.reshape(-1)]).to(dtype).contiguous()
    return (packed, mult.contiguous()) if normalize else packed


def stem_conv7(x, weight, bias, scale=None, out=None, relu=True, max_ctas=0):
    lib = _capi.load()
    _need(x, torch.float32, "stem_conv7 x", 4)
    _need16(weight, "stem_conv7 weight", 1)
    if weight.numel() != 7 * 8 * 64 * 8:
        raise ValueError(f"stem_conv7: weight must hold 28672 values (pack_stem_weight_fused), got {tuple(weight.shape)}")
    _need(bias, torch.float32, "stem_conv7 bias", 1)
    if scale is not None:
        _need(scale, torch.float32, "stem_conv7 scale", 1)
    if bias.shape[0] != 64 or (scale is not None and scale.shape[0] != 64):
        raise ValueError("stem_conv7: bias/scale must have 64 entries")
    n, d, h, w = x.shape
    shape = (n, (d - 1) // 2 + 1, (h - 1) // 2 + 1, (w - 1) // 2 + 1, 64)
    if out is None:
        out = torch.empty(shape, dtype=weight.dtype, device=x.device)
    _need(out, weight.dtype, "stem_conv7 out", 5)
    if tuple(out.shape) != shape:
        raise ValueError(f"stem_conv7: out shape {tuple(out.shape)} != {shape}")
    check(lib.dram_stem_conv7(_p(x), _p(weight), _p(bias), _p(scale), _p(out), n, d, h, w, 1 if relu else 0,
                              ACT_DTYPES[weight.dtype], max_ctas, _stream()), "dram_stem_conv7")
    return out


def stem_conv7_hu(hu, lut, weight, bias, scale=None, out=None, relu=True, lo=-1150, max_ctas=0):
    lib = _capi.load()
    _need(hu, torch.int16, "stem_conv7_hu hu", 4)
    _need(lut, torch.float32, "stem_conv7_hu lut", 2)
    _need16(weight, "stem_conv7_hu weight", 1)
    if weight.numel() != 7 * 8 * 64 * 8:
        raise ValueError("stem_conv7_hu: weight must hold 28672 values (pack_stem_weight_fused)")
    _need(bias, torch.float32, "stem_conv7_hu bias", 1)
    if scale is not None:
        _need(scale, torch.float32, "stem_conv7_hu scale", 1)
    n, d, h, w = hu.shape
    if lut.shape[0] != n:
        raise ValueError(f"stem_conv7_hu: lut must have {n} rows, got {tuple(lut.shape)}")
    shape = (n, (d - 1) // 2 + 1, (h - 1) // 2 + 1, (w - 1) // 2 + 1, 64)
    if out is None:
        out = torch.empty(shape, dtype=weight.dtype, device=hu.device)
    _need(out, weight.dtype, "stem_conv7_hu out", 5)
    if tuple(out.shape) != shape:
        raise ValueError(f"stem_conv7_hu: out shape {tuple(out.shape)} != {shape}")
    check(lib.dram_stem_conv7_hu(_p(hu), _p(lut), int(lo), lut.shape[1], _p(weight), _p(bias), _p(scale), _p(out), n, d,
                                 h, w, 1 if relu else 0, ACT_DTYPES[weight.dtype], max_ctas, _stream()),
          "dram_stem_conv7_hu")
    return out


def maxpool3d(x, out=None):
    _need16(x, "maxpool3d x", 5)
    n, d, h, w, c = x.shape
    shape = (n, (d - 1) // 2 + 1, (h - 1) // 2 + 1, (w - 1) // 2 + 1, c)
    if out is None:
        out = torch.empty(shape, dtype=x.dtype, device=x.device)
    _need(out, x.dtype, "maxpool3d out", 5)
    check(_capi.load().dram_maxpool3d(_p(x), _p(out), n, d, h, w, c, ACT_DTYPES[x.dtype], _stream()),
          "dram_maxpool3d")
    return out


def upsample2x(x, out=None):
    _need16(x, "upsample2x x", 5)
    n, d, h, w, c = x.shape
    if out is None:
        out = torch.empty((n, 2 * d, 2 * h, 2 * w, c), dtype=x.dtype, device=x.device)
    _need(out, x.dtype, "upsample2x out", 5)
    check(_capi.load().dram_upsample2x(_p(x), _p(out), n, d, h, w, c, ACT_DTYPES[x.dtype], _stream()),
          "dram_upsample2x")
    return out


class Upsample2xPlan:

    def __init__(self, x, out=None):
        lib = _capi.load()
        _need16(x, "upsample2x x", 5)
        n, d, h, w, c = x.shape
        if out is None:
            out = torch.empty((n, 2 * d, 2 * h, 2 * w, c), dtype=x.dtype, device=x.device)
        _need(out, x.dtype, "upsample2x out", 5)
        if tuple(out.shape) != (n, 2 * d, 2 * h, 2 * w, c):
            raise ValueError(f"upsample2x: out shape {tuple(out.shape)} does not match x {tuple(x.shape)}")
        handle = C.c_void_p()
        check(lib.dram_upsample2x_plan_create(_p(x), _p(out), n, d, h, w, c, ACT_DTYPES[x.dtype], C.byref(handle)),
              "dram_upsample2x_plan_create")
        self._handle, self._lib, self._keep, self.out = handle, lib, (x, out), out

    def run(self, max_ctas=0):
        check(self._lib.dram_upsample2x_plan_run(self._handle, max_ctas, _stream()), "dram_upsample2x_plan_run")
        return self.out

    def worklist_size(self):
        n = C.c_int32()
        check(self._lib.dram_upsample2x_worklist_size(self._handle, C.byref(n)), "dram_upsample2x_worklist_size")
        return n.value

    def build_worklist(self, support, radius, flags, items, count):
        check(self._lib.dram_upsample2x_worklist(self._handle, _p(support), radius, _p(flags), _p(items), _p(count),
                                                 _stream()), "dram_upsample2x_worklist")

    def run_listed(self, items, count, max_ctas=0):
        check(self._lib.dram_upsample2x_plan_run_listed(self._handle, _p(items), _p(count), max_ctas, _stream()),
              "dram_upsample2x_plan_run_listed")
        return self.out

    def __del__(self):
        h = getattr(self, "_handle", None)
        if h:
            try:
                self._lib.dram_upsample2x_plan_destroy(h)
            except Exception:
                pass
            self._handle = None


def decoder_support(ess, half_dims, rows=None, out=None):
    lib = _capi.load()
    _need(ess, torch.uint8, "decoder_support ess", 4)
    n, D, H, W = ess.shape
    d, h, w = half_dims
    words = (w + 31) // 32
    if rows is None:
        rows = torch.empty((n, D, H, words), dtype=torch.int32, device=ess.device)
    if out is None:
        out = torch.empty((n, d, h, words), dtype=torch.int32, device=ess.device)
    _need(rows, torch.int32, "decoder_support rows", 4)
    _need(out, torch.int32, "decoder_support out", 4)
    if tuple(rows.shape) != (n, D, H, words) or tuple(out.shape) != (n, d, h, words):
        raise ValueError("decoder_support: scratch / output shape mismatch")
    check(lib.dram_decoder_support(_p(ess), n, D, H, W, d, h, w, _p(rows), _p(out), _stream()), "dram_decoder_support")
    return out


def upconv_axis(x, axis, groups, out=None):
    _need16(x, "upconv_axis x", 5)
    if axis not in (1, 2, 3):
        raise ValueError("upconv_axis: axis must be 1 (D), 2 (H) or 3 (W)")
    n, d, h, w, c = x.shape
    if c < groups * 192:
        raise ValueError(f"upconv_axis: {c} channels cannot hold {groups} groups of 3 x 64")
    shape = [n, d, h, w, groups * 64]
    shape[axis] *= 2
    if out is None:
        out = torch.empty(shape, dtype=x.dtype, device=x.device)
    _need(out, x.dtype, "upconv_axis out", 5)
    if list(out.shape) != shape:
        raise ValueError(f"upconv_axis: out shape {tuple(out.shape)} != {tuple(shape)}")
    dims = (n, d, h, w)
    outer = 1
    for v in dims[:axis]:
        outer *= v
    inner = 1
    for v in dims[axis + 1:]:
        inner *= v
    check(_capi.load().dram_upconv_axis(_p(x), _p(out), outer, dims[axis], 2 * dims[axis], inner, groups, c,
                                        ACT_DTYPES[x.dtype], _stream()), "dram_upconv_axis")
    return out


def pack_upconv_weight(weight, c_up, scale=None, dtype=torch.bfloat16, pad_rows_to=256):
    w = weight.detach().to(torch.float32)[:, :c_up]
    if scale is not None:
        w = w * scale.to(torch.float32).view(-1, 1, 1, 1, 1)
    cout = w.shape[0]
    if cout != 64 or tuple(w.shape[2:]) != (3, 3, 3):
        raise ValueError(f"pack_upconv_weight: expected [64, C, 3, 3, 3], got {tuple(weight.shape)}")
    rows = w.reshape(cout, c_up, 27).permute(2, 0, 1).reshape(27 * cout, c_up)
    mult = pow2_normalizer(rows)
    packed = (rows / mult.view(-1, 1)).to(dtype)
    if pad_rows_to > 1 and packed.shape[0] % pad_rows_to:
        extra = pad_rows_to - packed.shape[0] % pad_rows_to
        packed = torch.cat([packed, packed.new_zeros((extra, c_up))])
        mult = torch.cat([mult, mult.new_ones(extra)])
    return packed.contiguous(), mult.contiguous()


def masked_pool(dense, mask=None):
    lib = _capi.load()
    _need(dense, torch.float32, "masked_pool dense", 5)
    n, ch, d, h, w = dense.shape
    md = mh = mw = 0
    is_f32 = 0
    if mask is not None:
        is_f32 = 1 if mask.dtype == torch.float32 else 0
        _need(mask, torch.float32 if is_f32 else torch.uint8, "masked_pool mask", 4)
        if mask.shape[0] != n:
            raise ValueError("masked_pool: mask batch mismatch")
        md, mh, mw = mask.shape[1:]
    ws = torch.empty(lib.dram_pool_workspace_bytes(n, ch), dtype=torch.uint8, device=dense.device)
    out = torch.empty((n, ch), dtype=torch.float32, device=dense.device)
    check(lib.dram_masked_pool(_p(dense), _p(mask), is_f32, _p(out), _p(ws), n, ch, d, h, w, md, mh, mw, _stream()),
          "dram_masked_pool")
    return out


def dram_upsample_mask(dense0, dense1, ess, lungs, size, per_sample_denominator=False, out=None):
    lib = _capi.load()
    _need(dense0, torch.float32, "dram dense0", 5)
    _need(dense1, torch.float32, "dram dense1", 5)
    _need(ess, torch.uint8, "dram ess", 4)
    _need(lungs, torch.uint8, "dram lungs", 4)
    n, ch, d, h, w = dense0.shape
    if ch != 1 or dense1.shape != dense0.shape:
        raise ValueError("dram_upsample_mask: dense maps must be [N,1,d,h,w] and alike")
    D, H, W = size
    if tuple(ess.shape) != (n, D, H, W) or tuple(lungs.shape) != (n, D, H, W):
        raise ValueError("dram_upsample_mask: mask shape mismatch")
    if out is None:
        out0 = torch.empty((n, 1, D, H, W), dtype=torch.float32, device=dense0.device)
        out1 = torch.empty_like(out0)
    else:
        out0, out1 = out
        _need(out0, torch.float32, "dram out0", 5)
        _need(out1, torch.float32, "dram out1", 5)
        if tuple(out0.shape) != (n, 1, D, H, W) or tuple(out1.shape) != (n, 1, D, H, W):
            raise ValueError("dram_upsample_mask: out tensors must be [N,1,D,H,W]")
    pct = torch.empty((2, n), dtype=torch.float32, device=dense0.device)
    ws = torch.empty(lib.dram_dram_workspace_bytes(n), dtype=torch.uint8, device=dense0.device)
    check(lib.dram_dram_upsample_mask(_p(dense0), _p(dense1), _p(ess), _p(lungs), _p(out0), _p(out1), _p(pct),
                                      _p(ws), n, d, h, w, D, H, W, 1 if per_sample_denominator else 0,
                                      _stream()), "dram_dram_upsample_mask")
    return out0, out1, pct


LOBE_LABELS = 256


def lobe_scores(cle, pse, ess, labels, out=None):
    lib = _capi.load()
    _need(cle, torch.float32, "lobe_scores cle", 5)
    _need(pse, torch.float32, "lobe_scores pse", 5)
    if isinstance(ess, torch.Tensor) and ess.dtype == torch.bool:
        ess = ess.view(torch.uint8)
    _need(ess, torch.uint8, "lobe_scores ess", 4)
    _need(labels, torch.uint8, "lobe_scores labels", 4)
    B, D, H, W = labels.shape
    if tuple(cle.shape) != (B, 1, D, H, W) or tuple(pse.shape) != (B, 1, D, H, W) or tuple(ess.shape) != (B, D, H, W):
        raise ValueError(f"lobe_scores: maps {tuple(cle.shape)} / {tuple(pse.shape)} and ess {tuple(ess.shape)} must "
                         f"match labels {tuple(labels.shape)}")
    if out is None:
        pct = torch.empty((2, B, LOBE_LABELS), dtype=torch.float32, device=labels.device)
        voxels = torch.empty((B, LOBE_LABELS), dtype=torch.int64, device=labels.device)
    else:
        pct, voxels = out
        _need(pct, torch.float32, "lobe_scores out pct", 3)
        _need(voxels, torch.int64, "lobe_scores out voxels", 2)
        if tuple(pct.shape) != (2, B, LOBE_LABELS) or tuple(voxels.shape) != (B, LOBE_LABELS):
            raise ValueError(f"lobe_scores: out must be ([2, {B}, 256], [{B}, 256])")
    count = D * H * W
    ws = torch.empty(lib.dram_lobe_workspace_bytes(B, count) // 8, dtype=torch.float64, device=labels.device)
    check(lib.dram_lobe_sums(_p(cle), _p(pse), _p(ess), _p(labels), _p(pct), _p(voxels), _p(ws), B, count, _stream()),
          "dram_lobe_sums")
    return pct, voxels


def window_standardize(hu, lo=-1150.0, hi=-300.0, out=None, batched=False):
    lib = _capi.load()
    _need(hu, torch.int16, "window_standardize hu")
    n = hu.shape[0] if batched else 1
    if out is None:
        out = torch.empty(hu.shape, dtype=torch.float32, device=hu.device)
    _need(out, torch.float32, "window_standardize out")
    stats = torch.empty((n, 2) if batched else (2,), dtype=torch.float32, device=hu.device)
    ws = torch.empty(lib.dram_preprocess_workspace_bytes_n(n) // 8, dtype=torch.float64, device=hu.device)
    check(lib.dram_window_standardize_batch(_p(hu), _p(out), _p(stats), _p(ws), n, hu.numel() // n, lo, hi, _stream()),
          "dram_window_standardize")
    return out, stats


def window_stats(hu, lo=-1150.0, hi=-300.0):
    lib = _capi.load()
    _need(hu, torch.int16, "window_stats hu")
    n = hu.shape[0]
    stats = torch.empty((n, 2), dtype=torch.float32, device=hu.device)
    ws = torch.empty(lib.dram_preprocess_workspace_bytes_n(n) // 8, dtype=torch.float64, device=hu.device)
    check(lib.dram_window_stats(_p(hu), _p(stats), _p(ws), n, hu.numel() // n, lo, hi, _stream()), "dram_window_stats")
    return stats


def window_lut(hu, lo=-1150, hi=-300):
    lib = _capi.load()
    _need(hu, torch.int16, "window_lut hu")
    if int(lo) != lo or int(hi) != hi:
        raise ValueError("window_lut: the window bounds must be integers")
    n = hu.shape[0]
    lut = torch.empty((n, int(hi) - int(lo) + 1), dtype=torch.float32, device=hu.device)
    stats = torch.empty((n, 2), dtype=torch.float32, device=hu.device)
    ws = torch.empty(lib.dram_preprocess_workspace_bytes_n(n) // 8, dtype=torch.float64, device=hu.device)
    check(lib.dram_window_lut(_p(hu), _p(lut), _p(stats), _p(ws), n, hu.numel() // n, float(lo), float(hi), _stream()),
          "dram_window_lut")
    return lut, stats


def slice_index(d_in, d_out, device):
    return torch.linspace(0, d_in - 1, d_out).long().to(torch.int32).to(device)


def resize_image(x, size):
    _need(x, torch.float32, "resize_image x", 3)
    D, H, W = x.shape
    D2, H2, W2 = size
    idx = slice_index(D, D2, x.device)
    out = torch.empty((D2, H2, W2), dtype=torch.float32, device=x.device)
    check(_capi.load().dram_resize_image(_p(x), _p(out), _p(idx), D, H, W, D2, H2, W2, _stream()),
          "dram_resize_image")
    return out


def resize_mask(x, size):
    _need(x, torch.uint8, "resize_mask x", 3)
    D, H, W = x.shape
    D2, H2, W2 = size
    idx = slice_index(D, D2, x.device)
    out = torch.empty((D2, H2, W2), dtype=torch.uint8, device=x.device)
    check(_capi.load().dram_resize_mask(_p(x), _p(out), _p(idx), D, H, W, D2, H2, W2, _stream()),
          "dram_resize_mask")
    return out


def resize_labels(x, size, out=None):
    _need(x, torch.uint8, "resize_labels x", 3)
    D, H, W = x.shape
    D2, H2, W2 = size
    idx = slice_index(D, D2, x.device)
    if out is None:
        out = torch.empty((D2, H2, W2), dtype=torch.uint8, device=x.device)
    _need(out, torch.uint8, "resize_labels out", 3)
    if tuple(out.shape) != (D2, H2, W2):
        raise ValueError(f"resize_labels: out shape {tuple(out.shape)} != {(D2, H2, W2)}")
    check(_capi.load().dram_resize_labels(_p(x), _p(out), _p(idx), D, H, W, D2, H2, W2, _stream()),
          "dram_resize_labels")
    return out


def mask_bbox(mask):
    _need(mask, torch.uint8, "mask_bbox mask", 3)
    D, H, W = mask.shape
    bbox = torch.empty(6, dtype=torch.int32, device=mask.device)
    check(_capi.load().dram_mask_bbox(_p(mask), D, H, W, _p(bbox), _stream()), "dram_mask_bbox")
    return bbox


def lung_crop(scan, lobe, crop, out=None):
    lib = _capi.load()
    _need(scan, torch.int16, "lung_crop scan", 3)
    _need(lobe, torch.uint8, "lung_crop lobe", 3)
    if scan.shape != lobe.shape:
        raise ValueError("scan and lobe segmentation have different shapes.")
    D, H, W = scan.shape
    (z0, z1), (y0, y1), (x0, x1) = [(int(a), int(b)) for a, b in crop]
    cd, ch, cw = z1 - z0, y1 - y0, x1 - x0
    if out is None:
        image = torch.empty((cd, ch, cw), dtype=torch.int16, device=scan.device)
        lung = torch.empty((cd, ch, cw), dtype=torch.uint8, device=scan.device)
        ess = torch.empty_like(lung)
    else:
        image, lung, ess = out
        _need(image, torch.int16, "lung_crop out image", 3)
        _need(lung, torch.uint8, "lung_crop out lung", 3)
        _need(ess, torch.uint8, "lung_crop out ess", 3)
        if not (tuple(image.shape) == tuple(lung.shape) == tuple(ess.shape) == (cd, ch, cw)):
            raise ValueError(f"lung_crop: out tensors must have the crop shape {(cd, ch, cw)}")
    ws = torch.empty(lib.dram_lung_crop_workspace_bytes(cd, ch, cw), dtype=torch.uint8, device=scan.device)
    check(lib.dram_lung_crop(_p(scan), _p(lobe), D, H, W, z0, y0, x0, cd, ch, cw, _p(image), _p(lung), _p(ess),
                             _p(ws), _stream()), "dram_lung_crop")
    return image, lung, ess


HU_BINS = 2048
HU_SLOTS = 16


def label_counts(labels):
    _need(labels, torch.uint8, "label_counts labels")
    counts = torch.empty(LOBE_LABELS, dtype=torch.int64, device=labels.device)
    check(_capi.load().dram_label_counts(_p(labels), labels.numel(), _p(counts), _stream()), "dram_label_counts")
    return counts


def hu_histograms(scan, labels, label_ids):
    lib = _capi.load()
    _need(scan, torch.int16, "hu_histograms scan")
    _need(labels, torch.uint8, "hu_histograms labels")
    if scan.shape != labels.shape:
        raise ValueError(f"hu_histograms: scan {tuple(scan.shape)} and labels {tuple(labels.shape)} differ in shape")
    ids = [int(k) for k in label_ids]
    if any(not 0 <= k < LOBE_LABELS for k in ids) or len(set(ids)) != len(ids):
        raise ValueError(f"hu_histograms: label ids must be distinct values in 0..255, got {ids}")
    hist = torch.empty((len(ids), HU_BINS), dtype=torch.int64, device=scan.device)
    hu_sum = torch.empty(len(ids), dtype=torch.int64, device=scan.device)
    for g in range(0, len(ids), HU_SLOTS):
        group = ids[g:g + HU_SLOTS]
        table = bytearray(b"\xff" * LOBE_LABELS)
        for s, k in enumerate(group):
            table[k] = s
        check(lib.dram_label_hu_hist(_p(scan), _p(labels), scan.numel(), bytes(table), len(group), _p(hist[g:]),
                                     _p(hu_sum[g:]), _stream()), "dram_label_hu_hist")
    return hist, hu_sum


def heatmap_u8(dram_map, crop, original_size, out=None):
    _need(dram_map, torch.float32, "heatmap_u8 map", 3)
    d, h, w = dram_map.shape
    OD, OH, OW = (int(v) for v in original_size)
    (z0, z1), (y0, y1), (x0, x1) = [(int(a), int(b)) for a, b in crop]
    if out is None:
        out = torch.empty((OD, OH, OW), dtype=torch.uint8, device=dram_map.device)
    _need(out, torch.uint8, "heatmap_u8 out", 3)
    check(_capi.load().dram_heatmap_u8(_p(dram_map), d, h, w, _p(out), OD, OH, OW, z0, y0, x0, z1 - z0, y1 - y0,
                                       x1 - x0, _stream()), "dram_heatmap_u8")
    return out


def to_ndhwc_16(x, dtype=torch.bfloat16):
    _need(x, torch.float32, "to_ndhwc_16 x", 5)
    n, c, d, h, w = x.shape
    out = torch.empty((n, d, h, w, c), dtype=dtype, device=x.device)
    check(_capi.load().dram_ncdhw_f32_to_ndhwc_16(_p(x), _p(out), n, c, d, h, w, ACT_DTYPES[dtype], _stream()),
          "dram_ncdhw_f32_to_ndhwc_16")
    return out


def to_ndhwc_bf16(x):
    return to_ndhwc_16(x, torch.bfloat16)


def to_ncdhw_f32(x):
    _need16(x, "to_ncdhw_f32 x", 5)
    n, d, h, w, c = x.shape
    out = torch.empty((n, c, d, h, w), dtype=torch.float32, device=x.device)
    check(_capi.load().dram_ndhwc_16_to_ncdhw_f32(_p(x), _p(out), n, c, d, h, w, ACT_DTYPES[x.dtype], _stream()),
          "dram_ndhwc_16_to_ncdhw_f32")
    return out


from . import custom_ops
```

### include/dram_b200.h

```cpp
#ifndef DRAM_B200_H_
#define DRAM_B200_H_

#include <stddef.h>
#include <stdint.h>

#ifdef __cplusplus
extern "C" {
#endif

#define DRAM_OK 0
#define DRAM_E_ARG (-1)
#define DRAM_E_ARCH (-2)
#define DRAM_E_LAUNCH (-3)
#define DRAM_E_DRIVER (-4)

#define DRAM_ABI_VERSION 5

#define DRAM_DTYPE_BF16 0
#define DRAM_DTYPE_F16 1

#define DRAM_CONV_ALGO_AUTO 0
#define DRAM_CONV_ALGO_TILES 1
#define DRAM_CONV_ALGO_PLANES 2
#define DRAM_CONV_EPILOGUE_AUTO 0
#define DRAM_CONV_EPILOGUE_DIRECT 1
#define DRAM_CONV_EPILOGUE_STAGED 2

int dram_version(void);
int dram_last_error(char *buf, size_t len);
int dram_sm_count(void);
int dram_set_saturation_counter(void *counter_u32);

typedef struct dram_conv_desc {
  int32_t n, di, hi, wi;
  int32_t c1;
  int32_t c2;
  int32_t cout;
  int32_t kd, kh, kw;
  int32_t sd, sh, sw;
  int32_t dd, dh, dw;
  int32_t pd, ph, pw;
  int32_t relu;
  int32_t res_c;
  int32_t res_stride;
  int32_t res_d, res_h, res_w;
  int32_t n_heads;
  int32_t head_ch[2];
  int32_t head_sigmoid;
  int32_t store_out;
  int32_t tw, th, td;
  int32_t dtype;
  int32_t algo;
  int32_t src1_up2x;
  int32_t epilogue;
} dram_conv_desc;

typedef struct dram_conv_plan dram_conv_plan;

int dram_conv3d_out_dims(const dram_conv_desc *d, int32_t *dout, int32_t *hout, int32_t *wout);

int dram_conv3d_plan_create(const dram_conv_desc *d, const void *src1, const void *src2,
                            const void *weight, const float *bias, const float *scale,
                            const void *residual, void *out, const float *head_w,
                            const float *head_b, float *head_out0, float *head_out1,
                            dram_conv_plan **plan);
int dram_conv3d_plan_destroy(dram_conv_plan *plan);
int dram_conv3d_run(const dram_conv_plan *plan, int32_t max_ctas, void *stream);
int dram_conv3d_plan_info(const dram_conv_plan *plan, int64_t *flops, int32_t *m_tiles,
                          int32_t *n_tiles, int32_t *block_n, int32_t *stages);
int dram_conv3d_plan_executed_flops(const dram_conv_plan *plan, int64_t *flops);
int dram_conv3d_worklist_size(const dram_conv_plan *plan, int32_t *entries);
int dram_conv3d_worklist(const dram_conv_plan *plan, const uint32_t *support, int32_t radius, uint8_t *flags,
                         int32_t *items, int32_t *count, void *stream);
int dram_conv3d_run_listed(const dram_conv_plan *plan, const int32_t *items, const int32_t *count, int32_t max_ctas,
                           void *stream);


int dram_stem_expand(const float *x, void *out, int32_t n, int32_t d, int32_t h, int32_t w,
                     int32_t dtype, void *stream);

size_t dram_stem_weight_bytes(void);
int dram_stem_conv7(const float *x, const void *weight, const float *bias, const float *scale,
                    void *out, int32_t n, int32_t d, int32_t h, int32_t w, int32_t relu,
                    int32_t dtype, int32_t max_ctas, void *stream);
#define DRAM_WINDOW_LUT_MAX 4096
int dram_stem_conv7_hu(const int16_t *hu, const float *lut, int32_t lut_lo, int32_t lut_size,
                       const void *weight, const float *bias, const float *scale, void *out, int32_t n,
                       int32_t d, int32_t h, int32_t w, int32_t relu, int32_t dtype, int32_t max_ctas,
                       void *stream);


int dram_maxpool3d(const void *x, void *out, int32_t n, int32_t d, int32_t h, int32_t w,
                   int32_t c, int32_t dtype, void *stream);

int dram_upsample2x(const void *x, void *out, int32_t n, int32_t d, int32_t h, int32_t w,
                    int32_t c, int32_t dtype, void *stream);

typedef struct dram_upsample_plan dram_upsample_plan;
int dram_upsample2x_plan_create(const void *x, void *out, int32_t n, int32_t d, int32_t h, int32_t w,
                                int32_t c, int32_t dtype, dram_upsample_plan **plan);
int dram_upsample2x_plan_destroy(dram_upsample_plan *plan);
int dram_upsample2x_plan_run(const dram_upsample_plan *plan, int32_t max_ctas, void *stream);
int dram_upsample2x_worklist_size(const dram_upsample_plan *plan, int32_t *entries);
int dram_upsample2x_worklist(const dram_upsample_plan *plan, const uint32_t *support, int32_t radius, uint8_t *flags,
                             int32_t *tiles, int32_t *count, void *stream);
int dram_upsample2x_plan_run_listed(const dram_upsample_plan *plan, const int32_t *tiles, const int32_t *count,
                                    int32_t max_ctas, void *stream);

int dram_decoder_support(const uint8_t *ess, int32_t n, int32_t D, int32_t H, int32_t W, int32_t d, int32_t h,
                         int32_t w, uint32_t *rows, uint32_t *support, void *stream);

int dram_upconv_axis(const void *in, void *out, int64_t outer, int32_t l_lo, int32_t l_hi, int64_t inner,
                     int32_t groups, int32_t in_channels, int32_t dtype, void *stream);

size_t dram_pool_workspace_bytes(int32_t n, int32_t ch);
int dram_masked_pool(const float *dense, const void *mask, int32_t mask_is_f32, float *out,
                     void *workspace, int32_t n, int32_t ch, int32_t d, int32_t h, int32_t w,
                     int32_t md, int32_t mh, int32_t mw, void *stream);

size_t dram_dram_workspace_bytes(int32_t n);
int dram_dram_upsample_mask(const float *dense0, const float *dense1, const uint8_t *ess,
                            const uint8_t *lungs, float *out0, float *out1, float *pct,
                            void *workspace, int32_t n, int32_t d, int32_t h, int32_t w,
                            int32_t D, int32_t H, int32_t W, int32_t per_sample_denominator,
                            void *stream);

size_t dram_lobe_workspace_bytes(int32_t n, int64_t count);
int dram_lobe_sums(const float *map0, const float *map1, const uint8_t *ess, const uint8_t *labels, float *pct,
                   int64_t *voxels, void *workspace, int32_t n, int64_t count, void *stream);

size_t dram_preprocess_workspace_bytes(void);
int dram_window_standardize(const int16_t *hu, float *out, float *stats_out, void *workspace,
                            int64_t count, float lo, float hi, void *stream);
size_t dram_preprocess_workspace_bytes_n(int32_t n);
int dram_window_standardize_batch(const int16_t *hu, float *out, float *stats_out, void *workspace,
                                  int32_t n, int64_t count, float lo, float hi, void *stream);
int dram_window_stats(const int16_t *hu, float *stats_out, void *workspace, int32_t n, int64_t count,
                      float lo, float hi, void *stream);
int dram_window_lut(const int16_t *hu, float *lut, float *stats_out, void *workspace, int32_t n,
                    int64_t count, float lo, float hi, void *stream);

int dram_resize_image(const float *x, float *out, const int32_t *d_idx, int32_t D, int32_t H,
                      int32_t W, int32_t D2, int32_t H2, int32_t W2, void *stream);
int dram_resize_mask(const uint8_t *x, uint8_t *out, const int32_t *d_idx, int32_t D, int32_t H,
                     int32_t W, int32_t D2, int32_t H2, int32_t W2, void *stream);
int dram_resize_labels(const uint8_t *x, uint8_t *out, const int32_t *d_idx, int32_t D, int32_t H,
                       int32_t W, int32_t D2, int32_t H2, int32_t W2, void *stream);

int dram_mask_bbox(const uint8_t *mask, int32_t D, int32_t H, int32_t W, int32_t *bbox, void *stream);
size_t dram_lung_crop_workspace_bytes(int32_t cd, int32_t ch, int32_t cw);
int dram_lung_crop(const int16_t *scan, const uint8_t *lobe, int32_t D, int32_t H, int32_t W, int32_t z0,
                   int32_t y0, int32_t x0, int32_t cd, int32_t ch, int32_t cw, int16_t *image_c,
                   uint8_t *lung_c, uint8_t *ess_c, void *workspace, void *stream);
int dram_label_counts(const uint8_t *labels, int64_t count, int64_t *counts, void *stream);
int dram_label_hu_hist(const int16_t *scan, const uint8_t *labels, int64_t count, const uint8_t *slot_of_label,
                       int32_t nslots, int64_t *hist, int64_t *hu_sum, void *stream);

int dram_heatmap_u8(const float *map, int32_t d, int32_t h, int32_t w, uint8_t *out, int32_t OD, int32_t OH,
                    int32_t OW, int32_t z0, int32_t y0, int32_t x0, int32_t cd, int32_t ch, int32_t cw,
                    void *stream);

typedef struct dram_wgrad_plan dram_wgrad_plan;
int64_t dram_conv3d_wgrad_workspace_bytes(const dram_conv_desc *d);
int dram_conv3d_wgrad_plan_create(const dram_conv_desc *d, const void *x, const void *dy, float *dw,
                                  int32_t cin_total, int32_t cin_offset, void *workspace,
                                  int64_t workspace_bytes, dram_wgrad_plan **plan);
int dram_conv3d_wgrad_plan_destroy(dram_wgrad_plan *plan);
int dram_conv3d_wgrad_plan_info(const dram_wgrad_plan *plan, int64_t *flops, int32_t *items, int32_t *kslices,
                                int32_t *block_n);
int dram_conv3d_wgrad_run(const dram_wgrad_plan *plan, int32_t accumulate, int32_t max_ctas, void *stream);

int64_t dram_bn_workspace_bytes(int32_t c);
int dram_bn_stats(const void *x, int64_t m, int32_t c, int32_t dtype, double *sums, void *workspace, void *stream);
int dram_bn_finalize(const double *sums, double count, const float *gamma, const float *beta, float eps,
                     float momentum, float *running_mean, float *running_var, float *scale, float *shift,
                     float *mean, float *rstd, int32_t c, void *stream);
int dram_bn_apply(const void *x, const float *scale, const float *shift, const void *res, int32_t relu, void *out,
                  int64_t m, int32_t c, int32_t dtype, void *stream);
int dram_bn_backward_reduce(const void *dy, const void *x, const void *y, const float *mean, const float *rstd,
                            int64_t m, int32_t c, int32_t dtype, double *sums, void *workspace, void *stream);
int dram_bn_backward_apply(const void *dy, const void *x, const void *y, const float *mean, const float *rstd,
                           const float *gamma, const double *sums, double count, void *dx, void *dres, int64_t m,
                           int32_t c, int32_t dtype, void *stream);

int dram_upsample2x_backward(const void *dy, void *dx, int32_t n, int32_t d, int32_t h, int32_t w, int32_t c,
                             int32_t dtype, void *stream);
int64_t dram_maxpool3d_backward_workspace_bytes(int32_t n, int32_t d, int32_t h, int32_t w, int32_t c);
int dram_maxpool3d_backward(const void *x, const void *dy, void *dx, void *workspace, int32_t n, int32_t d,
                            int32_t h, int32_t w, int32_t c, int32_t dtype, void *stream);

int64_t dram_heads_workspace_bytes(void);
int dram_heads_sigmoid_forward(const void *x, const float *w, const float *b, float *out0, float *out1, int64_t m,
                               int32_t dtype, void *stream);
int dram_heads_sigmoid_backward(const void *x, const float *w, const float *s0, const float *s1, const float *g0,
                                const float *g1, void *dx, float *dw, float *db, void *workspace, int64_t m,
                                int32_t dtype, void *stream);

#define DRAM_PEER_HANDLE_BYTES 64
int64_t dram_peer_exchange_bytes(void);
int dram_peer_alloc(int64_t bytes, void **ptr, void *handle64);
int dram_peer_open(const void *handle64, void **ptr);
int dram_peer_close(void *ptr);
int dram_peer_free(void *ptr);
int dram_peer_allreduce_f64(const double *in, double *out, int32_t n, void *const *peers, int32_t world, int32_t rank,
                            uint64_t seq, int32_t *status, void *stream);

#define DRAM_LOSS_COEF_TOTAL 0
#define DRAM_LOSS_COEF_CLE 1
#define DRAM_LOSS_COEF_PSE 2
#define DRAM_LOSS_COEF_MUL 3
#define DRAM_LOSS_COEF_SEG 4
#define DRAM_LOSS_COEF_HEAD 16
int64_t dram_train_loss_workspace_bytes(int32_t b);
int dram_train_loss_forward(const float *cle_map, const float *pse_map, const uint8_t *lungs, const uint8_t *ems,
                            const int64_t *cle_labels, const int64_t *pse_labels, const float *cle_bands,
                            const float *pse_bands, const float *cle_weights, const float *pse_weights, int32_t b,
                            int32_t d, int32_t h, int32_t w, int32_t d2, int32_t h2, int32_t w2, float beta,
                            float gamma, float *coef, void *workspace, void *stream);
int dram_train_loss_backward(const float *cle_map, const float *pse_map, const uint8_t *lungs, const uint8_t *ems,
                             const int64_t *cle_labels, const int64_t *pse_labels, const float *coef,
                             const float *grad_loss, int32_t b, int32_t d, int32_t h, int32_t w, int32_t d2,
                             int32_t h2, int32_t w2, float *grad_cle, float *grad_pse, void *stream);

int dram_adam_step(float *param, const float *grad, float *exp_avg, float *exp_avg_sq, int64_t n, double lr,
                   double beta1, double beta2, double eps, int32_t step, float grad_scale, void *stream);

int dram_pack_conv_weight(const float *w, void *out, int32_t cout, int32_t cin_total, int32_t taps, int32_t cin0,
                          int32_t cin_n, int32_t transpose, int32_t cout_pad, int32_t dtype, void *stream);

int dram_ncdhw_f32_to_ndhwc_16(const float *x, void *out, int32_t n, int32_t c, int32_t d,
                               int32_t h, int32_t w, int32_t dtype, void *stream);
int dram_ndhwc_16_to_ncdhw_f32(const void *x, float *out, int32_t n, int32_t c, int32_t d,
                               int32_t h, int32_t w, int32_t dtype, void *stream);

#ifdef __cplusplus
}
#endif
#endif
```

Baseline: 225.2.

## Group conv output positions into tap classes to skip padding taps exactly

New measurement: 233.0, median of 6. 1.03x the previous value.

```diff
diff --git a/bodyct-dram-emph-subtype_b200/_capi.py b/bodyct-dram-emph-subtype_b200/_capi.py
--- a/bodyct-dram-emph-subtype_b200/_capi.py
+++ b/bodyct-dram-emph-subtype_b200/_capi.py
@@ -36,6 +36,21 @@
     ]
 
 
+class ClassBox(C.Structure):
+
+    _fields_ = [("sample", C.c_int32), ("d0", C.c_int16), ("h0", C.c_int16), ("w0", C.c_int16),
+                ("shape", C.c_uint8), ("row0", C.c_uint8)]
+
+
+CLASS_MAX_BOXES = 8
+CLASS_MAX_SHAPES = 8
+
+
+class ClassTile(C.Structure):
+
+    _fields_ = [("taps", C.c_uint32), ("n_boxes", C.c_int32), ("box", ClassBox * CLASS_MAX_BOXES)]
+
+
 _vp, _i32, _i64, _sz = C.c_void_p, C.c_int32, C.c_int64, C.c_size_t
 _pi32 = C.POINTER(C.c_int32)
 
@@ -51,6 +66,7 @@
     "dram_conv3d_run": (C.c_int, [_vp, _i32, _vp]),
     "dram_conv3d_plan_info": (C.c_int, [_vp, C.POINTER(_i64), _pi32, _pi32, _pi32, _pi32]),
     "dram_conv3d_plan_executed_flops": (C.c_int, [_vp, C.POINTER(_i64)]),
+    "dram_conv3d_class_tiles": (C.c_int, [_i32, _i32, _i32, _i32, _i32, _i32, _vp, _i32, _pi32, _pi32, _pi32]),
     "dram_conv3d_worklist_size": (C.c_int, [_vp, _pi32]),
     "dram_conv3d_worklist": (C.c_int, [_vp, _vp, _i32, _vp, _vp, _vp, _vp]),
     "dram_conv3d_run_listed": (C.c_int, [_vp, _vp, _vp, _i32, _vp]),
diff --git a/bodyct-dram-emph-subtype_b200/csrc/conv3d_classes.cu b/bodyct-dram-emph-subtype_b200/csrc/conv3d_classes.cu
--- /dev/null
+++ b/bodyct-dram-emph-subtype_b200/csrc/conv3d_classes.cu
@@ -0,0 +1,194 @@
+#include <algorithm>
+#include <map>
+#include <mutex>
+#include <tuple>
+
+#include "conv_plan.h"
+
+namespace dram {
+
+namespace {
+
+struct Chunk {
+  int start, ext;
+};
+struct Segment {
+  uint32_t taps;
+  std::vector<Chunk> chunks;
+};
+
+uint32_t axis_taps(int o, int L, int dil) {
+  uint32_t m = 0;
+  for (int z = 0; z < 3; ++z) {
+    const int i = o + (z - 1) * dil;
+    if (i >= 0 && i < L) m |= 1u << z;
+  }
+  return m;
+}
+
+std::vector<Segment> axis_segments(int L, int dil, int max_ext) {
+  std::vector<Segment> segs;
+  for (int o = 0; o < L;) {
+    Segment s;
+    s.taps = axis_taps(o, L, dil);
+    int e = o + 1;
+    while (e < L && axis_taps(e, L, dil) == s.taps) ++e;
+    for (int x = o; x < e;) {
+      int c = max_ext;
+      while (c > e - x) c >>= 1;
+      s.chunks.push_back({x, c});
+      x += c;
+    }
+    segs.push_back(s);
+    o = e;
+  }
+  return segs;
+}
+
+bool build(int n, int D, int H, int W, int dil, bool pair, int max_w, ClassPlan *cp) {
+  const std::vector<Segment> sd = axis_segments(D, dil, 4), sh = axis_segments(H, dil, 4),
+                             sw = axis_segments(W, dil, max_w);
+  struct Cls {
+    uint32_t taps;
+    int a, b, c;
+  };
+  std::vector<Cls> classes;
+  for (int a = 0; a < (int)sd.size(); ++a)
+    for (int b = 0; b < (int)sh.size(); ++b)
+      for (int c = 0; c < (int)sw.size(); ++c) {
+        uint32_t taps = 0;
+        for (int zd = 0; zd < 3; ++zd)
+          for (int zh = 0; zh < 3; ++zh)
+            for (int zw = 0; zw < 3; ++zw)
+              if ((sd[a].taps >> zd & 1) && (sh[b].taps >> zh & 1) && (sw[c].taps >> zw & 1))
+                taps |= 1u << ((zd * 3 + zh) * 3 + zw);
+        classes.push_back({taps, a, b, c});
+      }
+#ifndef EXP_NO_SORT
+  std::stable_sort(classes.begin(), classes.end(),
+                   [](const Cls &x, const Cls &y) { return __builtin_popcount(x.taps) > __builtin_popcount(y.taps); });
+#endif
+
+  cp->tiles.clear();
+  cp->n_shapes = 0;
+  cp->stages = 0;
+  struct Box {
+    int rows;
+    dram_class_box b;
+  };
+  std::vector<Box> boxes;
+  for (const Cls &k : classes) {
+    boxes.clear();
+    for (int s = 0; s < n; ++s)
+      for (const Chunk &cd : sd[k.a].chunks)
+        for (const Chunk &ch : sh[k.b].chunks)
+          for (const Chunk &cw : sw[k.c].chunks) {
+            const int rows = cw.ext * ch.ext * cd.ext;
+            if (rows % 8 != 0) return false;
+            int shape = 0;
+            while (shape < cp->n_shapes && !(cp->shapes[shape][0] == cw.ext && cp->shapes[shape][1] == ch.ext &&
+                                             cp->shapes[shape][2] == cd.ext))
+              ++shape;
+            if (shape == cp->n_shapes) {
+              if (shape == DRAM_CLASS_MAX_SHAPES) return false;
+              cp->shapes[shape][0] = cw.ext;
+              cp->shapes[shape][1] = ch.ext;
+              cp->shapes[shape][2] = cd.ext;
+              ++cp->n_shapes;
+            }
+            Box bx;
+            memset(&bx.b, 0, sizeof(bx.b));
+            bx.rows = rows;
+            bx.b.sample = s;
+            bx.b.d0 = (int16_t)cd.start;
+            bx.b.h0 = (int16_t)ch.start;
+            bx.b.w0 = (int16_t)cw.start;
+            bx.b.shape = (uint8_t)shape;
+            boxes.push_back(bx);
+          }
+    std::stable_sort(boxes.begin(), boxes.end(), [](const Box &x, const Box &y) { return x.rows > y.rows; });
+    const size_t first = cp->tiles.size();
+    int used = 0;
+    for (const Box &bx : boxes) {
+      if (cp->tiles.size() == first || used + bx.rows > 128 || cp->tiles.back().n_boxes == DRAM_CLASS_MAX_BOXES) {
+        dram_class_tile t;
+        memset(&t, 0, sizeof(t));
+        t.taps = k.taps;
+        cp->tiles.push_back(t);
+        used = 0;
+      }
+      dram_class_tile &t = cp->tiles.back();
+      t.box[t.n_boxes] = bx.b;
+      t.box[t.n_boxes].row0 = (uint8_t)used;
+      ++t.n_boxes;
+      used += bx.rows;
+    }
+    if (pair && (cp->tiles.size() - first) % 2 == 1) {
+      dram_class_tile t;
+      memset(&t, 0, sizeof(t));
+      t.taps = k.taps;
+      cp->tiles.push_back(t);
+    }
+  }
+  for (const dram_class_tile &t : cp->tiles) cp->stages += __builtin_popcount(t.taps);
+  return true;
+}
+
+}
+
+bool class_plan_build(int n, int D, int H, int W, int dil, bool pair, ClassPlan *cp) {
+  if (n < 1 || D < 1 || H < 1 || W < 1 || dil < 1 || D > 32767 || H > 32767 || W > 32767) return false;
+  return build(n, D, H, W, dil, pair, 8, cp) || build(n, D, H, W, dil, pair, 4, cp);
+}
+
+int class_table_device(const ClassPlan &cp, int n, int D, int H, int W, int dil, bool pair,
+                       const dram_class_tile **table) {
+  static std::mutex mu;
+  static std::map<std::tuple<int, int, int, int, int, int, int>, dram_class_tile *> cache;
+  int dev = 0;
+  int rc = check_cuda(cudaGetDevice(&dev), "class tiles: cudaGetDevice");
+  if (rc != DRAM_OK) return rc;
+  std::lock_guard<std::mutex> lock(mu);
+  const auto key = std::make_tuple(dev, n, D, H, W, dil, (int)pair);
+  auto it = cache.find(key);
+  if (it != cache.end()) {
+    *table = it->second;
+    return DRAM_OK;
+  }
+  const size_t bytes = cp.tiles.size() * sizeof(dram_class_tile);
+  dram_class_tile *ptr = nullptr;
+  rc = check_cuda(cudaMalloc(&ptr, bytes), "class tiles: cudaMalloc");
+  if (rc != DRAM_OK) return rc;
+  rc = check_cuda(cudaMemcpy(ptr, cp.tiles.data(), bytes, cudaMemcpyHostToDevice), "class tiles: cudaMemcpy");
+  if (rc != DRAM_OK) {
+    cudaFree(ptr);
+    return rc;
+  }
+  cache[key] = ptr;
+  *table = ptr;
+  return DRAM_OK;
+}
+
+}
+
+extern "C" int dram_conv3d_class_tiles(int32_t n, int32_t d, int32_t h, int32_t w, int32_t dilation, int32_t pair,
+                                       dram_class_tile *tiles, int32_t capacity, int32_t *count, int32_t *shapes,
+                                       int32_t *n_shapes) {
+  DRAM_REQUIRE(count, "dram_conv3d_class_tiles: null count");
+  DRAM_REQUIRE(n > 0 && d > 0 && h > 0 && w > 0, "dram_conv3d_class_tiles: empty map %dx%dx%dx%d", n, d, h, w);
+  DRAM_REQUIRE(d <= 32767 && h <= 32767 && w <= 32767, "dram_conv3d_class_tiles: map extents must be <= 32767");
+  DRAM_REQUIRE(dilation >= 1, "dram_conv3d_class_tiles: dilation must be >= 1");
+  DRAM_REQUIRE(pair == 0 || pair == 1, "dram_conv3d_class_tiles: pair must be 0 or 1");
+  DRAM_REQUIRE(capacity >= 0, "dram_conv3d_class_tiles: negative capacity");
+  dram::ClassPlan cp;
+  if (!dram::class_plan_build(n, d, h, w, dilation, pair != 0, &cp)) cp.tiles.clear(), cp.n_shapes = 0;
+  DRAM_REQUIRE(!tiles || cp.tiles.size() <= (size_t)capacity, "dram_conv3d_class_tiles: %zu tiles, capacity %d",
+               cp.tiles.size(), capacity);
+  *count = (int32_t)cp.tiles.size();
+  if (tiles && !cp.tiles.empty()) memcpy(tiles, cp.tiles.data(), cp.tiles.size() * sizeof(dram_class_tile));
+  if (n_shapes) *n_shapes = cp.n_shapes;
+  if (shapes)
+    for (int i = 0; i < cp.n_shapes; ++i)
+      for (int j = 0; j < 3; ++j) shapes[3 * i + j] = cp.shapes[i][j];
+  return DRAM_OK;
+}
diff --git a/bodyct-dram-emph-subtype_b200/csrc/conv3d_pair.cu b/bodyct-dram-emph-subtype_b200/csrc/conv3d_pair.cu
--- a/bodyct-dram-emph-subtype_b200/csrc/conv3d_pair.cu
+++ b/bodyct-dram-emph-subtype_b200/csrc/conv3d_pair.cu
@@ -35,9 +35,11 @@
          tap_is_padding(t.w0 * p.sw + zw * p.dw - p.pw, p.tw, p.sw, p.Wi);
 }
 
+template <bool CLASS>
 __global__ void __launch_bounds__(P_THREADS, 1)
 conv3d_pair_kernel(const __grid_constant__ CUtensorMap map_a1, const __grid_constant__ CUtensorMap map_a2,
-                   const __grid_constant__ CUtensorMap map_w, const __grid_constant__ ConvKParams p) {
+                   const __grid_constant__ CUtensorMap map_w, const __grid_constant__ ActMaps<CLASS ? DRAM_CLASS_MAX_SHAPES : 1> cmaps,
+                   const __grid_constant__ ConvKParams p) {
   extern __shared__ uint8_t smem_raw[];
   const uint32_t smem_base = (smem_u32(smem_raw) + 1023u) & ~1023u;
   const uint32_t bar_base = smem_base + P_STAGES * P_STAGE_BYTES;
@@ -74,7 +76,32 @@
   asm volatile("ld.shared.b32 %0, [%1];" : "=r"(tmem_base) : "r"(tmem_slot));
   tmem_base = __shfl_sync(0xffffffffu, tmem_base, 0);
 
-  if (warp == P_PRODUCER_WARP) {
+  if (CLASS && warp == P_PRODUCER_WARP) {
+    if (lane == 0) {
+      int stage = 0;
+      uint32_t phase = 0;
+      for (int tile = blockIdx.x; tile < p.total_tiles; tile += gridDim.x) {
+        const int n0 = (tile % p.num_n_tiles) * P_BLOCK_N;
+        const dram_class_tile *ct = p.cls_tiles + 2 * (tile / p.num_n_tiles);
+        const uint32_t bytes = class_tile_bytes(p, ct) + class_tile_bytes(p, ct + 1) + P_B_BYTES;
+        for (uint32_t taps = ct->taps; taps != 0; taps &= taps - 1) {
+          const int tap = __ffs(taps) - 1;
+          for (int ch = 0; ch < p.chunks_total; ++ch) {
+            mbar_wait(empty_bar(stage), phase ^ 1u);
+            mbar_expect_tx(full_bar(stage), bytes);
+            for (int b = 0; b < 2; ++b)
+              class_tile_load(p, ct + b, cmaps.m, smem_a(stage, b), full_bar(stage), ch, tap / 9, tap / 3 % 3, tap % 3);
+            tma_load_2d(smem_b(stage), &map_w, full_bar(stage), (tap * p.chunks_total + ch) * P_BLOCK_K, n0);
+            if (++stage == P_STAGES) {
+              stage = 0;
+              phase ^= 1u;
+            }
+          }
+        }
+      }
+    }
+    __syncwarp();
+  } else if (warp == P_PRODUCER_WARP) {
     if (lane == 0) {
       int stage = 0;
       uint32_t phase = 0;
@@ -115,36 +142,42 @@
     int stage = 0;
     uint32_t phase = 0, acc_phase = 0;
     for (int tile = blockIdx.x; tile < p.total_tiles; tile += gridDim.x) {
-      const PairCoord pc = decode_pair(p, tile);
       mbar_wait(tmem_empty_bar, acc_phase ^ 1u);
       tcgen05_fence_after();
       uint32_t accumulate = 0;
-      for (int zd = 0; zd < p.kd; ++zd)
-        for (int zh = 0; zh < p.kh; ++zh)
-          for (int zw = 0; zw < p.kw; ++zw) {
-            if (brick_tap_is_padding(p, pc.t[0], zd, zh, zw) && brick_tap_is_padding(p, pc.t[1], zd, zh, zw)) continue;
-            for (int ch = 0; ch < p.chunks_total; ++ch) {
-              mbar_wait(full_bar(stage), phase);
-              tcgen05_fence_after();
-              const uint64_t da0 = make_sw128_desc(smem_a(stage, 0)), da1 = make_sw128_desc(smem_a(stage, 1));
-              const uint64_t db = make_sw128_desc(smem_b(stage));
-              if (elect_one_sync()) {
+      auto issue_tap = [&]() {
+        for (int ch = 0; ch < p.chunks_total; ++ch) {
+          mbar_wait(full_bar(stage), phase);
+          tcgen05_fence_after();
+          const uint64_t da0 = make_sw128_desc(smem_a(stage, 0)), da1 = make_sw128_desc(smem_a(stage, 1));
+          const uint64_t db = make_sw128_desc(smem_b(stage));
+          if (elect_one_sync()) {
 #pragma unroll
-                for (int k = 0; k < 4; ++k) {
-                  umma_bf16(tmem_base, da0 + (uint64_t)(2 * k), db + (uint64_t)(2 * k), idesc, (k > 0) ? 1u : accumulate);
-                  umma_bf16(tmem_base + P_BLOCK_N, da1 + (uint64_t)(2 * k), db + (uint64_t)(2 * k), idesc,
-                            (k > 0) ? 1u : accumulate);
-                }
-                umma_commit(empty_bar(stage));
-              }
-              __syncwarp();
-              accumulate = 1;
-              if (++stage == P_STAGES) {
-                stage = 0;
-                phase ^= 1u;
-              }
+            for (int k = 0; k < 4; ++k) {
+              umma_bf16(tmem_base, da0 + (uint64_t)(2 * k), db + (uint64_t)(2 * k), idesc, (k > 0) ? 1u : accumulate);
+              umma_bf16(tmem_base + P_BLOCK_N, da1 + (uint64_t)(2 * k), db + (uint64_t)(2 * k), idesc,
+                        (k > 0) ? 1u : accumulate);
             }
+            umma_commit(empty_bar(stage));
           }
+          __syncwarp();
+          accumulate = 1;
+          if (++stage == P_STAGES) {
+            stage = 0;
+            phase ^= 1u;
+          }
+        }
+      };
+      if (CLASS) {
+        for (uint32_t taps = p.cls_tiles[2 * (tile / p.num_n_tiles)].taps; taps != 0; taps &= taps - 1) issue_tap();
+      } else {
+        const PairCoord pc = decode_pair(p, tile);
+        for (int zd = 0; zd < p.kd; ++zd)
+          for (int zh = 0; zh < p.kh; ++zh)
+            for (int zw = 0; zw < p.kw; ++zw)
+              if (!(brick_tap_is_padding(p, pc.t[0], zd, zh, zw) && brick_tap_is_padding(p, pc.t[1], zd, zh, zw)))
+                issue_tap();
+      }
       if (elect_one_sync()) umma_commit(tmem_full_bar);
       __syncwarp();
       acc_phase ^= 1u;
@@ -157,10 +190,21 @@
     const int ld = row >> (p.tw_log2 + p.th_log2);
     uint32_t acc_phase = 0;
     for (int tile = blockIdx.x; tile < p.total_tiles; tile += gridDim.x) {
-      const PairCoord pc = decode_pair(p, tile);
-      const TileCoord &t = pc.t[brick];
-      const int od = t.d0 + ld, oh = t.h0 + lh, ow = t.w0 + lw;
-      const bool valid = pc.m_ok[brick] && (od < p.Do) && (oh < p.Ho) && (ow < p.Wo);
+      TileCoord t;
+      int od, oh, ow;
+      bool valid;
+      if (CLASS) {
+        const ClassRow cr = class_row(p, p.cls_tiles + 2 * (tile / p.num_n_tiles) + brick, row);
+        t.n0 = (tile % p.num_n_tiles) * P_BLOCK_N;
+        t.sample = cr.sample;
+        od = cr.od, oh = cr.oh, ow = cr.ow;
+        valid = cr.valid;
+      } else {
+        const PairCoord pc = decode_pair(p, tile);
+        t = pc.t[brick];
+        od = t.d0 + ld, oh = t.h0 + lh, ow = t.w0 + lw;
+        valid = pc.m_ok[brick] && (od < p.Do) && (oh < p.Ho) && (ow < p.Wo);
+      }
       const uint16_t *res_row = residual_row(p.epi, valid, t.sample, od, oh, ow);
       mbar_wait(tmem_full_bar, acc_phase);
       tcgen05_fence_after();
@@ -198,23 +242,34 @@
   return k_chunks >= 200 && pair_tiles >= 6LL * sm_count();
 }
 
-int pair_plan_fill(dram_conv_plan *pl) {
+int pair_plan_fill(dram_conv_plan *pl, int m_tiles) {
   ConvKParams &p = pl->p;
-  p.m_tiles_total = pl->m_tiles;
-  const int64_t total = (int64_t)((pl->m_tiles + 1) / 2) * p.num_n_tiles;
+  p.m_tiles_total = m_tiles;
+  const int64_t total = (int64_t)((m_tiles + 1) / 2) * p.num_n_tiles;
   p.total_tiles = (int)total;
   pl->pair = 1;
   pl->stages = P_STAGES;
   pl->smem_bytes = P_SMEM_BYTES;
-  return check_cuda(cudaFuncSetAttribute(conv3d_pair_kernel, cudaFuncAttributeMaxDynamicSharedMemorySize, P_SMEM_BYTES),
+  return check_cuda(pl->cls ? cudaFuncSetAttribute(conv3d_pair_kernel<true>, cudaFuncAttributeMaxDynamicSharedMemorySize,
+                                                   P_SMEM_BYTES)
+                            : cudaFuncSetAttribute(conv3d_pair_kernel<false>,
+                                                   cudaFuncAttributeMaxDynamicSharedMemorySize, P_SMEM_BYTES),
                     "cudaFuncSetAttribute(conv3d_pair_kernel)");
+}
+
+template <bool CLASS>
+static void launch_pair(const dram_conv_plan *pl, int ctas, cudaStream_t st) {
+  ConvKParams kp = pl->p;
+  kp.epi = with_sat_counter(kp.epi);
+  ActMaps<CLASS ? DRAM_CLASS_MAX_SHAPES : 1> cmaps;
+  memcpy(&cmaps, &pl->cls_maps, sizeof(cmaps));
+  conv3d_pair_kernel<CLASS><<<ctas, P_THREADS, pl->smem_bytes, st>>>(pl->map_a1, pl->map_a2, pl->map_w, cmaps, kp);
 }
 
 int pair_plan_run(const dram_conv_plan *pl, int ctas, cudaStream_t st) {
   if (pl->p.total_tiles < ctas) ctas = pl->p.total_tiles;
-  ConvKParams kp = pl->p;
-  kp.epi = with_sat_counter(kp.epi);
-  conv3d_pair_kernel<<<ctas, P_THREADS, pl->smem_bytes, st>>>(pl->map_a1, pl->map_a2, pl->map_w, kp);
+  if (pl->cls) launch_pair<true>(pl, ctas, st);
+  else launch_pair<false>(pl, ctas, st);
   DRAM_CHECK_LAUNCH("conv3d_pair_kernel launch");
   return DRAM_OK;
 }
diff --git a/bodyct-dram-emph-subtype_b200/csrc/conv3d_umma.cu b/bodyct-dram-emph-subtype_b200/csrc/conv3d_umma.cu
--- a/bodyct-dram-emph-subtype_b200/csrc/conv3d_umma.cu
+++ b/bodyct-dram-emph-subtype_b200/csrc/conv3d_umma.cu
@@ -26,12 +26,12 @@
   static constexpr int SMEM_BYTES = 1024 + STAGES * STAGE_BYTES + EPI_BYTES + 256;
 };
 
-template <int BLOCK_N, bool STAGED>
-__global__ void __launch_bounds__(STAGED ? NUM_THREADS_STAGED : NUM_THREADS, 1)
-conv3d_umma_kernel(const __grid_constant__ CUtensorMap map_a1,
-                   const __grid_constant__ CUtensorMap map_a2,
-                   const __grid_constant__ CUtensorMap map_w, const __grid_constant__ CUtensorMap map_out,
-                   const __grid_constant__ CUtensorMap map_res, const __grid_constant__ ConvKParams p) {
+template <int BLOCK_N, bool STAGED, bool CLASS>
+__device__ __forceinline__ void conv3d_umma_body(const CUtensorMap &map_a1, const CUtensorMap &map_a2,
+                                                 const CUtensorMap &map_w, const CUtensorMap &map_out,
+                                                 const CUtensorMap &map_res, const CUtensorMap *cmaps,
+                                                 const ConvKParams &p) {
+  static_assert(!(STAGED && CLASS), "class tiles use the direct epilogue");
   using Cfg = ConvCfg<BLOCK_N, STAGED>;
   constexpr int STAGES = Cfg::STAGES;
   extern __shared__ uint8_t smem_raw[];
@@ -82,7 +82,33 @@
   asm volatile("ld.shared.b32 %0, [%1];" : "=r"(tmem_base) : "r"(tmem_slot));
   tmem_base = __shfl_sync(0xffffffffu, tmem_base, 0);
 
-  if (warp == PRODUCER_WARP) {
+  if (CLASS && warp == PRODUCER_WARP) {
+    if (lane == 0) {
+      int stage = 0;
+      uint32_t phase = 0;
+      for (int tile = blockIdx.x; tile < p.total_tiles; tile += gridDim.x) {
+        const int n0 = (tile % p.num_n_tiles) * BLOCK_N;
+        const dram_class_tile *ct = p.cls_tiles + tile / p.num_n_tiles;
+        ClassLoads L;
+        class_tile_fetch(p, ct, L);
+        const uint32_t bytes = L.bytes + Cfg::B_STAGE_BYTES;
+        for (uint32_t taps = ct->taps; taps != 0; taps &= taps - 1) {
+          const int tap = __ffs(taps) - 1;
+          for (int ch = 0; ch < p.chunks_total; ++ch) {
+            mbar_wait(empty_bar(stage), phase ^ 1u);
+            mbar_expect_tx(full_bar(stage), bytes);
+            class_tile_load(p, L, cmaps, smem_a(stage), full_bar(stage), ch, tap / 9, tap / 3 % 3, tap % 3);
+            tma_load_2d(smem_b(stage), &map_w, full_bar(stage), (tap * p.chunks_total + ch) * BLOCK_K, n0);
+            if (++stage == STAGES) {
+              stage = 0;
+              phase ^= 1u;
+            }
+          }
+        }
+      }
+    }
+    __syncwarp();
+  } else if (warp == PRODUCER_WARP) {
     if (lane == 0) {
       int stage = 0;
       uint32_t phase = 0;
@@ -128,36 +154,42 @@
       int acc = 0;
       uint32_t acc_phase = 0;
       for (int tile = blockIdx.x; tile < p.total_tiles; tile += gridDim.x) {
-        const TileCoord t = decode_tile(p, tile, BLOCK_N);
         mbar_wait(tmem_empty_bar(acc), acc_phase ^ 1u);
         tcgen05_fence_after();
         const uint32_t tmem_d = tmem_base + (uint32_t)(acc * BLOCK_N);
         uint32_t accumulate = 0;
-        for (int zd = 0; zd < p.kd; ++zd) {
-          if (tap_is_padding(t.d0 * p.sd + zd * p.dd - p.pd, p.td, p.sd, p.Di)) continue;
-          for (int zh = 0; zh < p.kh; ++zh) {
-            if (tap_is_padding(t.h0 * p.sh + zh * p.dh - p.ph, p.th, p.sh, p.Hi)) continue;
-            for (int zw = 0; zw < p.kw; ++zw) {
-              if (tap_is_padding(t.w0 * p.sw + zw * p.dw - p.pw, p.tw, p.sw, p.Wi)) continue;
-              for (int ch = 0; ch < p.chunks_total; ++ch) {
-                mbar_wait(full_bar(stage), phase);
-                tcgen05_fence_after();
-                const uint64_t da = make_sw128_desc(smem_a(stage));
-                const uint64_t db = make_sw128_desc(smem_b(stage));
-                if (elect_one_sync()) {
+        auto issue_tap = [&]() {
+          for (int ch = 0; ch < p.chunks_total; ++ch) {
+            mbar_wait(full_bar(stage), phase);
+            tcgen05_fence_after();
+            const uint64_t da = make_sw128_desc(smem_a(stage));
+            const uint64_t db = make_sw128_desc(smem_b(stage));
+            if (elect_one_sync()) {
 #pragma unroll
-                  for (int k = 0; k < BLOCK_K / UMMA_K; ++k) {
-                    umma_bf16(tmem_d, da + (uint64_t)(2 * k), db + (uint64_t)(2 * k), idesc,
-                              (k > 0) ? 1u : accumulate);
-                  }
-                  umma_commit(empty_bar(stage));
-                }
-                __syncwarp();
-                accumulate = 1;
-                if (++stage == STAGES) {
-                  stage = 0;
-                  phase ^= 1u;
-                }
+              for (int k = 0; k < BLOCK_K / UMMA_K; ++k) {
+                umma_bf16(tmem_d, da + (uint64_t)(2 * k), db + (uint64_t)(2 * k), idesc, (k > 0) ? 1u : accumulate);
+              }
+              umma_commit(empty_bar(stage));
+            }
+            __syncwarp();
+            accumulate = 1;
+            if (++stage == STAGES) {
+              stage = 0;
+              phase ^= 1u;
+            }
+          }
+        };
+        if (CLASS) {
+          for (uint32_t taps = p.cls_tiles[tile / p.num_n_tiles].taps; taps != 0; taps &= taps - 1) issue_tap();
+        } else {
+          const TileCoord t = decode_tile(p, tile, BLOCK_N);
+          for (int zd = 0; zd < p.kd; ++zd) {
+            if (tap_is_padding(t.d0 * p.sd + zd * p.dd - p.pd, p.td, p.sd, p.Di)) continue;
+            for (int zh = 0; zh < p.kh; ++zh) {
+              if (tap_is_padding(t.h0 * p.sh + zh * p.dh - p.ph, p.th, p.sh, p.Hi)) continue;
+              for (int zw = 0; zw < p.kw; ++zw) {
+                if (tap_is_padding(t.w0 * p.sw + zw * p.dw - p.pw, p.tw, p.sw, p.Wi)) continue;
+                issue_tap();
               }
             }
           }
@@ -238,9 +270,20 @@
     int acc = 0;
     uint32_t acc_phase = 0;
     for (int tile = blockIdx.x; tile < p.total_tiles; tile += gridDim.x) {
-      const TileCoord t = decode_tile(p, tile, BLOCK_N);
-      const int od = t.d0 + ld, oh = t.h0 + lh, ow = t.w0 + lw;
-      const bool valid = (od < p.Do) && (oh < p.Ho) && (ow < p.Wo);
+      TileCoord t;
+      int od, oh, ow;
+      bool valid;
+      if (CLASS) {
+        const ClassRow cr = class_row(p, p.cls_tiles + tile / p.num_n_tiles, row);
+        t.n0 = (tile % p.num_n_tiles) * BLOCK_N;
+        t.sample = cr.sample;
+        od = cr.od, oh = cr.oh, ow = cr.ow;
+        valid = cr.valid;
+      } else {
+        t = decode_tile(p, tile, BLOCK_N);
+        od = t.d0 + ld, oh = t.h0 + lh, ow = t.w0 + lw;
+        valid = (od < p.Do) && (oh < p.Ho) && (ow < p.Wo);
+      }
       const uint16_t *res_row = residual_row(p.epi, valid, t.sample, od, oh, ow);
       ResGroup res = load_residual_group(p.epi, res_row, t.n0);
       mbar_wait(tmem_full_bar(acc), acc_phase);
@@ -270,6 +313,22 @@
     tcgen05_fence_after();
     tmem_dealloc(tmem_base, Cfg::TMEM_COLS);
   }
+}
+
+template <int BLOCK_N, bool STAGED>
+__global__ void __launch_bounds__(STAGED ? NUM_THREADS_STAGED : NUM_THREADS, 1)
+conv3d_umma_kernel(const __grid_constant__ CUtensorMap map_a1,
+                   const __grid_constant__ CUtensorMap map_a2,
+                   const __grid_constant__ CUtensorMap map_w, const __grid_constant__ CUtensorMap map_out,
+                   const __grid_constant__ CUtensorMap map_res, const __grid_constant__ ConvKParams p) {
+  conv3d_umma_body<BLOCK_N, STAGED, false>(map_a1, map_a2, map_w, map_out, map_res, nullptr, p);
+}
+
+template <int BLOCK_N>
+__global__ void __launch_bounds__(NUM_THREADS, 1)
+conv3d_class_kernel(const __grid_constant__ CUtensorMap map_w, const __grid_constant__ ClassMaps cmaps,
+                    const __grid_constant__ ConvKParams p) {
+  conv3d_umma_body<BLOCK_N, false, true>(map_w, map_w, map_w, map_w, map_w, cmaps.m, p);
 }
 
 typedef CUresult (*EncodeTiledFn)(CUtensorMap *, CUtensorMapDataType, cuuint32_t, void *,
@@ -370,7 +429,7 @@
 static int conv_out(int in, int k, int s, int d, int p) { return (in + 2 * p - d * (k - 1) - 1) / s + 1; }
 
 int pair_plan_wanted(const dram_conv_desc *d, int block_n, int64_t k_chunks, int64_t m_tiles, int n_tiles);
-int pair_plan_fill(dram_conv_plan *pl);
+int pair_plan_fill(dram_conv_plan *pl, int m_tiles);
 int pair_plan_run(const dram_conv_plan *pl, int ctas, cudaStream_t st);
 
 int slab_plan_supported(const dram_conv_desc *d);
@@ -395,25 +454,100 @@
   return DRAM_OK;
 }
 
-template <int BN, bool STAGED>
-static int set_smem_attr() {
-  return check_cuda(cudaFuncSetAttribute(conv3d_umma_kernel<BN, STAGED>,
-                                         cudaFuncAttributeMaxDynamicSharedMemorySize,
-                                         ConvCfg<BN, STAGED>::SMEM_BYTES),
-                    "cudaFuncSetAttribute(conv3d_umma_kernel)");
-}
-template <int BN, bool STAGED>
+template <int BN, bool STAGED, bool CLASS = false>
 static int fill_tile_cfg(dram_conv_plan *pl) {
   pl->stages = ConvCfg<BN, STAGED>::STAGES;
   pl->smem_bytes = ConvCfg<BN, STAGED>::SMEM_BYTES;
-  return set_smem_attr<BN, STAGED>();
-}
-template <int BN, bool STAGED>
+  return CLASS ? check_cuda(cudaFuncSetAttribute(conv3d_class_kernel<BN>, cudaFuncAttributeMaxDynamicSharedMemorySize,
+                                                 ConvCfg<BN, false>::SMEM_BYTES),
+                            "cudaFuncSetAttribute(conv3d_class_kernel)")
+               : check_cuda(cudaFuncSetAttribute(conv3d_umma_kernel<BN, STAGED>,
+                                                 cudaFuncAttributeMaxDynamicSharedMemorySize,
+                                                 ConvCfg<BN, STAGED>::SMEM_BYTES),
+                            "cudaFuncSetAttribute(conv3d_umma_kernel)");
+}
+template <int BN, bool STAGED, bool CLASS = false>
 static void launch_tiles(const dram_conv_plan *pl, dim3 grid, cudaStream_t st) {
   ConvKParams kp = pl->p;
   kp.epi = with_sat_counter(kp.epi);
-  conv3d_umma_kernel<BN, STAGED><<<grid, STAGED ? NUM_THREADS_STAGED : NUM_THREADS, pl->smem_bytes, st>>>(
-      pl->map_a1, pl->map_a2, pl->map_w, pl->map_out, pl->map_res, kp);
+  if (CLASS)
+    conv3d_class_kernel<BN><<<grid, NUM_THREADS, pl->smem_bytes, st>>>(pl->map_w, pl->cls_maps, kp);
+  else
+    conv3d_umma_kernel<BN, STAGED><<<grid, STAGED ? NUM_THREADS_STAGED : NUM_THREADS, pl->smem_bytes, st>>>(
+        pl->map_a1, pl->map_a2, pl->map_w, pl->map_out, pl->map_res, kp);
+}
+
+static bool host_tap_is_padding(int i0, int extent, int stride, int in_size) {
+  return (i0 + (extent - 1) * stride < 0) || (i0 >= in_size);
+}
+static bool host_brick_tap_skipped(const ConvKParams &p, int m_tile, int zd, int zh, int zw) {
+  const int r = m_tile % p.tiles_per_sample;
+  const int iw = r % p.tiles_w, r2 = r / p.tiles_w, ih = r2 % p.tiles_h, id = r2 / p.tiles_h;
+  return host_tap_is_padding(id * p.td * p.sd + zd * p.dd - p.pd, p.td, p.sd, p.Di) ||
+         host_tap_is_padding(ih * p.th * p.sh + zh * p.dh - p.ph, p.th, p.sh, p.Hi) ||
+         host_tap_is_padding(iw * p.tw * p.sw + zw * p.dw - p.pw, p.tw, p.sw, p.Wi);
+}
+static int64_t raster_stages(const ConvKParams &p, int m_tiles, bool pair) {
+  int64_t stages = 0;
+  if (pair) {
+    for (int pr = 0; 2 * pr < m_tiles; ++pr)
+      for (int zd = 0; zd < p.kd; ++zd)
+        for (int zh = 0; zh < p.kh; ++zh)
+          for (int zw = 0; zw < p.kw; ++zw) {
+            const bool s0 = host_brick_tap_skipped(p, 2 * pr, zd, zh, zw);
+            const bool s1 = 2 * pr + 1 < m_tiles ? host_brick_tap_skipped(p, 2 * pr + 1, zd, zh, zw) : true;
+            if (!(s0 && s1)) stages += 2;
+          }
+  } else {
+    for (int m = 0; m < m_tiles; ++m)
+      for (int zd = 0; zd < p.kd; ++zd)
+        for (int zh = 0; zh < p.kh; ++zh)
+          for (int zw = 0; zw < p.kw; ++zw)
+            if (!host_brick_tap_skipped(p, m, zd, zh, zw)) ++stages;
+  }
+  return stages;
+}
+
+static int class_plan_fill(dram_conv_plan *pl, const dram_conv_desc *d, const void *src1, int64_t k_chunks,
+                           bool *used) {
+  *used = false;
+  ConvKParams &p = pl->p;
+  const bool shape_ok = d->tw == 0 && d->c2 == 0 && d->kd == 3 && d->kh == 3 && d->kw == 3 && d->sd == 1 &&
+                        d->sh == 1 && d->sw == 1 && d->dd == d->dh && d->dd == d->dw && d->pd == d->dd &&
+                        d->ph == d->dh && d->pw == d->dw;
+  ClassPlan cp;
+  if (!shape_ok || !class_plan_build(d->n, p.Do, p.Ho, p.Wo, d->dd, false, &cp)) return DRAM_OK;
+  const bool pair = pair_plan_wanted(d, pl->block_n, k_chunks, (int64_t)cp.tiles.size(), pl->n_tiles);
+  if (pair && !class_plan_build(d->n, p.Do, p.Ho, p.Wo, d->dd, true, &cp)) return DRAM_OK;
+  const bool raster_pair = pair_plan_wanted(d, pl->block_n, k_chunks, pl->m_tiles, pl->n_tiles);
+  if (cp.stages >= raster_stages(p, pl->m_tiles, raster_pair)) return DRAM_OK;
+  if ((int64_t)cp.tiles.size() * pl->n_tiles > 0x7fffffffLL) return DRAM_OK;
+
+  const dram_class_tile *table = nullptr;
+  int rc = class_table_device(cp, d->n, p.Do, p.Ho, p.Wo, d->dd, pair, &table);
+  for (int s = 0; rc == DRAM_OK && s < cp.n_shapes; ++s) {
+    rc = encode_act_map(&pl->cls_maps.m[s], src1, d->n, d->di, d->hi, d->wi, d->c1, BLOCK_K, cp.shapes[s][0],
+                        cp.shapes[s][1], cp.shapes[s][2], 1, 1, 1, p.epi.is_f16);
+    for (int a = 0; a < 3; ++a) p.cls_log2[s][a] = (uint8_t)ilog2(cp.shapes[s][a]);
+  }
+  if (rc != DRAM_OK) return rc;
+  p.cls_tiles = table;
+  pl->cls = 1;
+  pl->cls_stages = cp.stages;
+  const int tiles = (int)cp.tiles.size();
+  if (pair) {
+    rc = pair_plan_fill(pl, tiles);
+  } else {
+    p.total_tiles = tiles * pl->n_tiles;
+    switch (pl->block_n) {
+      case 32: rc = fill_tile_cfg<32, false, true>(pl); break;
+      case 64: rc = fill_tile_cfg<64, false, true>(pl); break;
+      case 128: rc = fill_tile_cfg<128, false, true>(pl); break;
+      default: rc = fill_tile_cfg<256, false, true>(pl); break;
+    }
+  }
+  *used = rc == DRAM_OK;
+  return rc;
 }
 
 extern "C" int dram_conv3d_plan_create(const dram_conv_desc *d, const void *src1, const void *src2,
@@ -622,14 +756,20 @@
         case 256: rc = fill_tile_cfg<256, true>(pl); break;
         default: rc = fill_tile_cfg<128, true>(pl); break;
       }
-    } else if (d->tw == 0 && pair_plan_wanted(d, block_n, (int64_t)taps * p.chunks_total, pl->m_tiles, pl->n_tiles)) {
-      rc = pair_plan_fill(pl);
     } else {
-      switch (block_n) {
-        case 32: rc = fill_tile_cfg<32, false>(pl); break;
-        case 64: rc = fill_tile_cfg<64, false>(pl); break;
-        case 128: rc = fill_tile_cfg<128, false>(pl); break;
-        default: rc = fill_tile_cfg<256, false>(pl); break;
+      bool cls = false;
+      rc = class_plan_fill(pl, d, src1, (int64_t)taps * p.chunks_total, &cls);
+      if (rc == DRAM_OK && !cls) {
+        if (d->tw == 0 && pair_plan_wanted(d, block_n, (int64_t)taps * p.chunks_total, pl->m_tiles, pl->n_tiles)) {
+          rc = pair_plan_fill(pl, pl->m_tiles);
+        } else {
+          switch (block_n) {
+            case 32: rc = fill_tile_cfg<32, false>(pl); break;
+            case 64: rc = fill_tile_cfg<64, false>(pl); break;
+            case 128: rc = fill_tile_cfg<128, false>(pl); break;
+            default: rc = fill_tile_cfg<256, false>(pl); break;
+          }
+        }
       }
     }
   }
@@ -657,16 +797,6 @@
   return DRAM_OK;
 }
 
-static bool host_tap_is_padding(int i0, int extent, int stride, int in_size) {
-  return (i0 + (extent - 1) * stride < 0) || (i0 >= in_size);
-}
-static bool host_brick_tap_skipped(const ConvKParams &p, int m_tile, int zd, int zh, int zw) {
-  const int r = m_tile % p.tiles_per_sample;
-  const int iw = r % p.tiles_w, r2 = r / p.tiles_w, ih = r2 % p.tiles_h, id = r2 / p.tiles_h;
-  return host_tap_is_padding(id * p.td * p.sd + zd * p.dd - p.pd, p.td, p.sd, p.Di) ||
-         host_tap_is_padding(ih * p.th * p.sh + zh * p.dh - p.ph, p.th, p.sh, p.Hi) ||
-         host_tap_is_padding(iw * p.tw * p.sw + zw * p.dw - p.pw, p.tw, p.sw, p.Wi);
-}
 
 extern "C" int dram_conv3d_plan_executed_flops(const dram_conv_plan *plan, int64_t *flops) {
   DRAM_REQUIRE(plan && flops, "dram_conv3d_plan_executed_flops: null argument");
@@ -682,24 +812,7 @@
     return DRAM_OK;
   }
   const ConvKParams &p = plan->p;
-  const int m_tiles = plan->m_tiles;
-  int64_t stages = 0;
-  if (plan->pair) {
-    for (int pr = 0; 2 * pr < m_tiles; ++pr)
-      for (int zd = 0; zd < p.kd; ++zd)
-        for (int zh = 0; zh < p.kh; ++zh)
-          for (int zw = 0; zw < p.kw; ++zw) {
-            const bool s0 = host_brick_tap_skipped(p, 2 * pr, zd, zh, zw);
-            const bool s1 = 2 * pr + 1 < m_tiles ? host_brick_tap_skipped(p, 2 * pr + 1, zd, zh, zw) : true;
-            if (!(s0 && s1)) stages += 2;
-          }
-  } else {
-    for (int m = 0; m < m_tiles; ++m)
-      for (int zd = 0; zd < p.kd; ++zd)
-        for (int zh = 0; zh < p.kh; ++zh)
-          for (int zw = 0; zw < p.kw; ++zw)
-            if (!host_brick_tap_skipped(p, m, zd, zh, zw)) ++stages;
-  }
+  const int64_t stages = plan->cls ? plan->cls_stages : raster_stages(p, plan->m_tiles, plan->pair != 0);
   *flops = 2LL * stages * p.num_n_tiles * 128 * (int64_t)plan->block_n * p.chunks_total * 64;
   return DRAM_OK;
 }
@@ -713,7 +826,14 @@
   if (plan->pair) return pair_plan_run(plan, ctas, st);
   if (plan->p.total_tiles < ctas) ctas = plan->p.total_tiles;
   dim3 grid(ctas);
-  if (plan->staged) {
+  if (plan->cls) {
+    switch (plan->block_n) {
+      case 32: launch_tiles<32, false, true>(plan, grid, st); break;
+      case 64: launch_tiles<64, false, true>(plan, grid, st); break;
+      case 128: launch_tiles<128, false, true>(plan, grid, st); break;
+      default: launch_tiles<256, false, true>(plan, grid, st); break;
+    }
+  } else if (plan->staged) {
     switch (plan->block_n) {
       case 64: launch_tiles<64, true>(plan, grid, st); break;
       case 256: launch_tiles<256, true>(plan, grid, st); break;
@@ -727,7 +847,7 @@
       default: launch_tiles<256, false>(plan, grid, st); break;
     }
   }
-  DRAM_CHECK_LAUNCH("conv3d_umma_kernel launch");
+  DRAM_CHECK_LAUNCH(plan->cls ? "conv3d_class_kernel launch" : "conv3d_umma_kernel launch");
   return DRAM_OK;
 }
 
diff --git a/bodyct-dram-emph-subtype_b200/csrc/conv_plan.h b/bodyct-dram-emph-subtype_b200/csrc/conv_plan.h
--- a/bodyct-dram-emph-subtype_b200/csrc/conv_plan.h
+++ b/bodyct-dram-emph-subtype_b200/csrc/conv_plan.h
@@ -1,7 +1,15 @@
 #pragma once
+#include <vector>
+
 #include "umma_common.cuh"
 
 namespace dram {
+
+template <int N>
+struct ActMaps {
+  CUtensorMap m[N];
+};
+using ClassMaps = ActMaps<DRAM_CLASS_MAX_SHAPES>;
 
 struct ConvKParams {
   int n, Do, Ho, Wo, Di, Hi, Wi;
@@ -12,8 +20,20 @@
   int chunks1, chunks_total;
   int staged_res;
   int m_tiles_total;
+  const dram_class_tile *cls_tiles;
+  uint8_t cls_log2[DRAM_CLASS_MAX_SHAPES][3];
   EpiParams epi;
 };
+
+struct ClassPlan {
+  std::vector<dram_class_tile> tiles;
+  int shapes[DRAM_CLASS_MAX_SHAPES][3];
+  int n_shapes;
+  int64_t stages;
+};
+bool class_plan_build(int n, int D, int H, int W, int dil, bool pair, ClassPlan *cp);
+int class_table_device(const ClassPlan &cp, int n, int D, int H, int W, int dil, bool pair,
+                       const dram_class_tile **table);
 
 
 #ifdef __CUDACC__
@@ -39,6 +59,78 @@
 __device__ __forceinline__ bool tap_is_padding(int i0, int extent, int stride, int in_size) {
   return (i0 + (extent - 1) * stride < 0) || (i0 >= in_size);
 }
+struct ClassRow {
+  bool valid;
+  int sample, od, oh, ow;
+};
+__device__ __forceinline__ ClassRow class_row(const ConvKParams &p, const dram_class_tile *ct, int row) {
+  ClassRow r = {false, 0, 0, 0, 0};
+  const int nb = ct->n_boxes;
+  for (int b = 0; b < nb; ++b) {
+    const dram_class_box bx = ct->box[b];
+    const int lw = p.cls_log2[bx.shape][0], lh = p.cls_log2[bx.shape][1], ld = p.cls_log2[bx.shape][2];
+    const int i = row - bx.row0;
+    if (i >= 0 && i < (1 << (lw + lh + ld))) {
+      r.valid = true;
+      r.sample = bx.sample;
+      r.ow = bx.w0 + (i & ((1 << lw) - 1));
+      r.oh = bx.h0 + ((i >> lw) & ((1 << lh) - 1));
+      r.od = bx.d0 + (i >> (lw + lh));
+    }
+  }
+  return r;
+}
+__device__ __forceinline__ uint32_t class_tile_bytes(const ConvKParams &p, const dram_class_tile *ct) {
+  uint32_t rows = 0;
+  const int nb = ct->n_boxes;
+  for (int b = 0; b < nb; ++b) {
+    const int s = ct->box[b].shape;
+    rows += 1u << (p.cls_log2[s][0] + p.cls_log2[s][1] + p.cls_log2[s][2]);
+  }
+  return rows * 128u;
+}
+__device__ __forceinline__ void class_tile_load(const ConvKParams &p, const dram_class_tile *ct,
+                                                const CUtensorMap *maps, uint32_t smem_a, uint32_t bar, int ch,
+                                                int zd, int zh, int zw) {
+  const int nb = ct->n_boxes;
+  for (int b = 0; b < nb; ++b) {
+    const dram_class_box bx = ct->box[b];
+    tma_load_5d(smem_a + (uint32_t)bx.row0 * 128u, maps + bx.shape, bar, ch * 64, bx.w0 + zw * p.dw - p.pw,
+                bx.h0 + zh * p.dh - p.ph, bx.d0 + zd * p.dd - p.pd, bx.sample);
+  }
+}
+struct ClassLoads {
+  int n;
+  uint32_t bytes;
+  uint32_t meta[DRAM_CLASS_MAX_BOXES];
+  uint32_t wh[DRAM_CLASS_MAX_BOXES];
+  int d[DRAM_CLASS_MAX_BOXES], s[DRAM_CLASS_MAX_BOXES];
+};
+__device__ __forceinline__ void class_tile_fetch(const ConvKParams &p, const dram_class_tile *ct, ClassLoads &L) {
+  L.n = ct->n_boxes;
+  L.bytes = 0;
+#pragma unroll
+  for (int b = 0; b < DRAM_CLASS_MAX_BOXES; ++b) {
+    if (b < L.n) {
+      const dram_class_box bx = ct->box[b];
+      const int sh = bx.shape;
+      L.meta[b] = (uint32_t)bx.row0 * 128u | (uint32_t)sh << 16;
+      L.wh[b] = (uint32_t)(uint16_t)(bx.w0 - p.pw) | (uint32_t)(bx.h0 - p.ph) << 16;
+      L.d[b] = bx.d0 - p.pd;
+      L.s[b] = bx.sample;
+      L.bytes += 128u << (p.cls_log2[sh][0] + p.cls_log2[sh][1] + p.cls_log2[sh][2]);
+    }
+  }
+}
+__device__ __forceinline__ void class_tile_load(const ConvKParams &p, const ClassLoads &L, const CUtensorMap *maps,
+                                                uint32_t smem_a, uint32_t bar, int ch, int zd, int zh, int zw) {
+  const int ow = zw * p.dw, oh = zh * p.dh, od = zd * p.dd;
+#pragma unroll
+  for (int b = 0; b < DRAM_CLASS_MAX_BOXES; ++b)
+    if (b < L.n)
+      tma_load_5d(smem_a + (L.meta[b] & 0xffffu), maps + (L.meta[b] >> 16), bar, ch * 64, (int)(int16_t)L.wh[b] + ow,
+                  ((int)L.wh[b] >> 16) + oh, L.d[b] + od, L.s[b]);
+}
 #endif
 
 struct SlabParams {
@@ -63,6 +155,9 @@
   CUtensorMap map_out, map_res;
   int staged;
   int pair;
+  int cls;
+  int64_t cls_stages;
+  dram::ClassMaps cls_maps;
   dram::ConvKParams p;
   dram::SlabParams sp;
   int block_n;
diff --git a/bodyct-dram-emph-subtype_b200/ops.py b/bodyct-dram-emph-subtype_b200/ops.py
--- a/bodyct-dram-emph-subtype_b200/ops.py
+++ b/bodyct-dram-emph-subtype_b200/ops.py
@@ -201,6 +201,18 @@
             self._handle = None
 
 
+def class_tiles(n, d, h, w, dilation, pair=False):
+    lib = _capi.load()
+    count, n_shapes = C.c_int32(), C.c_int32()
+    check(lib.dram_conv3d_class_tiles(n, d, h, w, dilation, int(pair), None, 0, C.byref(count), None, None),
+          "dram_conv3d_class_tiles")
+    tiles = (_capi.ClassTile * max(count.value, 1))()
+    shapes = (C.c_int32 * (3 * _capi.CLASS_MAX_SHAPES))()
+    check(lib.dram_conv3d_class_tiles(n, d, h, w, dilation, int(pair), tiles, count.value, C.byref(count), shapes,
+                                      C.byref(n_shapes)), "dram_conv3d_class_tiles")
+    return list(tiles[:count.value]), [tuple(shapes[3 * i:3 * i + 3]) for i in range(n_shapes.value)]
+
+
 def pow2_normalizer(w2d):
     amax = w2d.abs().amax(dim=1).clamp_min(2.0 ** -100)
     return torch.exp2(torch.floor(torch.log2(amax)) + 1.0)
diff --git a/include/dram_b200.h b/include/dram_b200.h
--- a/include/dram_b200.h
+++ b/include/dram_b200.h
@@ -69,6 +69,23 @@
 int dram_conv3d_plan_info(const dram_conv_plan *plan, int64_t *flops, int32_t *m_tiles,
                           int32_t *n_tiles, int32_t *block_n, int32_t *stages);
 int dram_conv3d_plan_executed_flops(const dram_conv_plan *plan, int64_t *flops);
+#define DRAM_CLASS_MAX_BOXES 8
+#ifndef DRAM_CLASS_MAX_SHAPES
+#define DRAM_CLASS_MAX_SHAPES 8
+#endif
+typedef struct {
+  int32_t sample;
+  int16_t d0, h0, w0;
+  uint8_t shape, row0;
+} dram_class_box;
+typedef struct {
+  uint32_t taps;
+  int32_t n_boxes;
+  dram_class_box box[DRAM_CLASS_MAX_BOXES];
+} dram_class_tile;
+int dram_conv3d_class_tiles(int32_t n, int32_t d, int32_t h, int32_t w, int32_t dilation, int32_t pair,
+                            dram_class_tile *tiles, int32_t capacity, int32_t *count, int32_t *shapes,
+                            int32_t *n_shapes);
 int dram_conv3d_worklist_size(const dram_conv_plan *plan, int32_t *entries);
 int dram_conv3d_worklist(const dram_conv_plan *plan, const uint32_t *support, int32_t radius, uint8_t *flags,
                          int32_t *items, int32_t *count, void *stream);
```
